# nianticlabs/map-free-reloc

Hardware: AMD Instinct MI355X
Metric: image-pairs/sec @ 540x720 (SuperPoint+SuperGlue + PnP w/ depth) (higher is better)
Workload: dtype f32 in / f32 accumulate; matrix products of the 3x3 convolutions, attention, the transformer's linear layers and SuperPoint's 1x1 descriptor head on the f16 matrix cores with every fp32 operand carried as TWO f16 terms (xh = rne_f16(x), xl = rne_f16((x - xh) 2^11); weights pre-scaled per output feat

## Files before the change

include/mfr_hip.h:

```cpp
#ifndef MFR_HIP_H
#define MFR_HIP_H
#include <stddef.h>
#include <stdint.h>

#ifdef __cplusplus
extern "C" {
#endif

#define MFR_ABI_VERSION 6

#define MFR_K_F32 0
#define MFR_K_F64 1

#define MFR_E_ARG      (-1)
#define MFR_E_LAUNCH   (-2)
#define MFR_E_WORKSPACE (-3)

#define MFR_ST_OK          0
#define MFR_ST_TOO_FEW     1
#define MFR_ST_BAD_DEPTH   2
#define MFR_ST_NO_MODEL    3
#define MFR_ST_DEGENERATE  4

int mfr_abi_version(void);

int mfr_f16x2_guard_bind(int *device_flag);
#define MFR_ST_RANGE 7
const char *mfr_target_arch(void);

int mfr_test_f64_ops(const double *a, const double *b, const double *c, int n, double *out3, void *stream);
int mfr_test_sample(uint64_t seed, const int64_t *pair_ids, int B, int iters, int n, int k, int32_t *out, void *stream);

size_t mfr_pnp_workspace_bytes(int B, int maxN, int max_iters);
int mfr_pnp_solve_batch(const float *pts0, const float *pts1, const int32_t *n_corr, int B, int maxN,
                        const float *depth0, int H, int W,
                        const void *K0, const void *K1, int k_dtype,
                        int max_iters, double reproj_thr, double confidence,
                        uint64_t seed, const int64_t *pair_ids,
                        void *workspace, size_t workspace_bytes,
                        double *R, double *t, int32_t *n_inliers, int32_t *status, uint8_t *inlier_mask,
                        void *stream);

int mfr_depth_min(const float *depth, int B, int H, int W, float *partial_min , void *stream);
int mfr_pnp_lift(const float *pts0, const float *pts1, const int32_t *n_corr, int B, int maxN,
                 const float *depth0, const float *partial_min, int H, int W, const void *K0, int k_dtype,
                 double *xyz, double *obs, int32_t *src_idx, int32_t *n_valid, void *stream);
int mfr_pnp_ransac(const double *xyz, const double *obs, const int32_t *n_valid, int B, int maxN,
                   const void *K1, int k_dtype, int max_iters, double reproj_thr, double confidence,
                   uint64_t seed, const int64_t *pair_ids,
                   int32_t *counts , int32_t *inl_idx ,
                   double *R, double *t, int32_t *n_inliers, int32_t *status,
                   uint8_t *mask_valid ,
                   int32_t *best_iter , int32_t *iters_run ,
                   void *stream);

size_t mfr_rig_pnp_workspace_bytes(int B, int T, int maxN, int max_iters);
int mfr_rig_pnp_ransac(const double *xyz, const double *obs, const int32_t *n_valid, int B, int T, int maxN,
                       const void *K1, int k_dtype, const double *rig, int max_iters, double reproj_thr, double confidence,
                       uint64_t seed, const int64_t *pair_ids,
                       int32_t *counts , int32_t *inl_idx ,
                       double *R, double *t, int32_t *n_inliers, int32_t *status,
                       uint8_t *mask_valid ,
                       int32_t *best_iter , int32_t *iters_run ,
                       void *stream);
int mfr_rig_pnp_solve_batch(const float *pts0, const float *pts1, const int32_t *n_corr, int B, int T, int maxN,
                            const float *depth0, int H, int W,
                            const void *K0, const void *K1, int k_dtype, const double *rig,
                            int max_iters, double reproj_thr, double confidence,
                            uint64_t seed, const int64_t *pair_ids,
                            void *workspace, size_t workspace_bytes,
                            double *R, double *t, int32_t *n_inliers, int32_t *status, uint8_t *inlier_mask ,
                            void *stream);

size_t mfr_scale_workspace_bytes(int B, int maxN);
int mfr_scale_from_depth_batch(const float *pts0, const float *pts1, const uint8_t *emat_mask,
                               const int32_t *n_corr, int B, int maxN,
                               const float *depth0, const float *depth1, int H, int W,
                               const void *K0, const void *K1, int k_dtype,
                               const double *R, const double *t,
                               const int32_t *in_status ,
                               double scale_thr,
                               void *workspace, size_t workspace_bytes,
                               double *t_metric, double *best_scale, int32_t *n_inliers, int32_t *status,
                               void *stream);

#define MFR_AP_OK            0
#define MFR_AP_APPROXIMATED  1
#define MFR_AP_NO_PAIRS      2
#define MFR_AP_TOO_MANY      3
#define MFR_AP_BAD_OFFSETS   4
#define MFR_AP_ITER_CAP      16
#define MFR_AP_MAX_PAIRS     64
#define MFR_AP_MAX_LO_ITERS  62
#define MFR_AP_WEISZFELD_CAP 256
size_t mfr_abs_pose_workspace_bytes(int P);
int mfr_abs_pose_fuse(const double *train_q, const double *train_c, const double *pred_R, const double *pred_t, int P,
                      const int32_t *offsets, int Q, int mode, double thr_deg, double thr_mult, int lo_iters, uint64_t seed,
                      void *workspace, size_t workspace_bytes,
                      double *abs_q, double *abs_c, int32_t *inlier_mask, int32_t *status, void *stream);
int mfr_test_abs_pose_subset(uint64_t seed, const uint64_t *base, int n, int calls, int iters, int nsub, uint64_t *out, void *stream);

#define MFR_EMAT_SCORE_MAGSAC 0
#define MFR_EMAT_SCORE_COUNT  1
#define MFR_MAGSAC_LUT_M 2048
int mfr_magsac_lut(double *lut_host , int M);
size_t mfr_emat_workspace_bytes(int B, int maxN, int max_iters);
int mfr_emat_solve_batch(const float *pts0, const float *pts1, const int32_t *n_corr, int B, int maxN,
                         const void *K0, const void *K1, int k_dtype, double pix_thr, double confidence, int max_iters,
                         uint64_t seed, const int64_t *pair_ids, int score_method, const double *magsac_lut, int lut_m,
                         double max_thr_ratio, void *workspace, size_t workspace_bytes,
                         double *R, double *t, int32_t *n_inliers, int32_t *status, uint8_t *inlier_mask,
                         int32_t *best_iter, int32_t *iters_run, int32_t *counts_out, double *losses_out, int32_t *lo_runs,
                         void *stream);

size_t mfr_procrustes_workspace_bytes(int B, int maxN, int max_iters);
int mfr_procrustes_solve_batch(const float *pts0, const float *pts1, const int32_t *n_corr, int B, int maxN,
                               const float *depth0, const float *depth1, int H, int W, const void *K0, const void *K1, int k_dtype,
                               double max_corr_dist, double confidence, int max_iters, uint64_t seed, const int64_t *pair_ids,
                               void *workspace, size_t workspace_bytes, double *R, double *t, int32_t *n_inliers,
                               int32_t *status, int32_t *best_iter, int32_t *iters_run, int32_t *counts_out, void *stream);

int mfr_sp_scoremap(const float *logits, int B, int Hc, int Wc, float *scores, void *stream);
int mfr_sp_nms_candidates(const float *scores, int B, int H, int W, int nms_radius, float threshold, int border,
                          float *nms_out, uint64_t *cand, int cand_cap, int32_t *cand_count, void *stream);
int mfr_sp_nms_candidates_variant(const float *scores, int B, int H, int W, int nms_radius, float threshold, int border,
                                  float *nms_out, uint64_t *cand, int cand_cap, int32_t *cand_count, int variant, void *stream);
int mfr_sp_nms_stream_geometry(int *useful_cols, int *segment_rows);
int mfr_sp_select_topk(const uint64_t *cand, int cand_cap, const int32_t *cand_count, int B, int W, int K,
                       float *kpts, float *kscores, int32_t *n_kpts, void *stream);
int mfr_sp_sample_descriptors(const float *dense_nhwc, int B, int Hc, int Wc, const float *kpts,
                              const int32_t *n_kpts, int K, float *desc, void *stream);
int mfr_sp_sample_descriptors_ld(const float *dense_nhwc, int B, int Hc, int Wc, const float *kpts,
                                 const int32_t *n_kpts, int K, float *desc, int ldd, void *stream);

size_t mfr_gemm_f16x2_pack_bytes(int N, int K);
int mfr_gemm_f16x2_pack(const float *w, int N, int K, void *packed, void *stream);
int mfr_gemm_f16x2(const float *x, int ldx, const void *packed_w, const float *bias, float *y, int ldy, int M, int N, int K, int flags, void *stream);
int mfr_gemm_f16x2_pack_batched(const float *w, int ldw, int nbatch, long long w_batch_stride, int N, int K, float out_mul, void *packed, void *stream);
int mfr_gemm_f16x2_batched(const float *x, int ldx, long long x_batch_stride, const void *packed_w, const float *bias, float *y, int ldy, long long y_batch_stride,
                           int nbatch, int M, int N, int K, int flags, void *stream);
int mfr_conv_igemm_k(int Cin, int KH, int KW);
int mfr_conv_igemm_f16x2(const float *x, const void *packed_w, const float *bias, float *y, int B, int Cin, int H, int W, int Cout, int KH, int KW,
                         int stride, int pad, int relu, void *stream);
int mfr_conv_igemm_f16x2_pad(const float *x, const void *packed_w, const float *bias, float *y, int B, int Cin, int H, int W, int Cout, int KH, int KW,
                             int stride, int pad_lo, int pad_hi, int relu, void *stream);
int mfr_conv_igemm_f16x2_upadd(const float *x, const void *packed_w, const float *bias, const float *lo, int Hl, int Wl, float *y, int B, int Cin, int H, int W,
                               int Cout, int KH, int KW, int stride, int pad, void *stream);
int mfr_gemm_f16x2_ln(const float *x, int ldx, const void *packed_w, const float *bias, const float *gamma, const float *beta, float eps, float *y, int ldy,
                      int M, int N, int K, int accumulate, void *stream);
int mfr_gemm_bf16x3_ln(const float *x, int ldx, const void *packed_w, const float *bias, const float *gamma, const float *beta, float eps, float *y, int ldy,
                       int M, int N, int K, int accumulate, void *stream);
int mfr_gemm_f16x2_windows(const float *feat, int Bimg, int Hf, int Wf, int C, const int32_t *img_ids, const int32_t *cell_ids, int nwin, int wc, int stride, int win,
                           const float *zero_row, const void *packed_w, const float *bias, const float *window_bias, float *y, int ldy, int N, void *stream);
int mfr_gemm_bf16x3_windows(const float *feat, int Bimg, int Hf, int Wf, int C, const int32_t *img_ids, const int32_t *cell_ids, int nwin, int wc, int stride, int win,
                            const float *zero_row, const void *packed_w, const float *bias, const float *window_bias, float *y, int ldy, int N, void *stream);
int mfr_mlp_ln_f16x2(const float *x, int ldx, int K1, const void *packed_w1, const float *b1, const void *packed_w2, const float *b2, const float *gamma, const float *beta,
                     float eps, float *y, int ldy, int M, int accumulate, void *stream);
int mfr_mlp_ln_bf16x3(const float *x, int ldx, int K1, const void *packed_w1, const float *b1, const void *packed_w2, const float *b2, const float *gamma, const float *beta,
                      float eps, float *y, int ldy, int M, int accumulate, void *stream);
size_t mfr_gemm_bf16x3_pack_bytes(int N, int K);
int mfr_gemm_bf16x3_pack(const float *w, int N, int K, void *packed, void *stream);
int mfr_gemm_bf16x3(const float *x, int ldx, const void *packed_w, const float *bias, float *y, int ldy, int M, int N, int K, int flags, void *stream);
int mfr_sg_attention(const float *q, const float *k, const float *v, int ld, int B2, int N, int heads,
                     const int32_t *n_tok, int cross, float *out, int ldo, void *stream);
int mfr_sg_attention_variant(const float *q, const float *k, const float *v, int ld, int B2, int N, int heads,
                             const int32_t *n_tok, int cross, float *out, int ldo, int variant, void *stream);
size_t mfr_sg_match_workspace_bytes(int B, int ldS);
int mfr_sg_sinkhorn_match(const float *S, int B, int ldS, const int32_t *n0, const int32_t *n1,
                          float bin_score, int iters, float match_thr,
                          const float *kpts0, const float *kpts1, int K,
                          void *workspace, size_t workspace_bytes,
                          int32_t *matches0, float *mscores0, float *pts0, float *pts1, int maxN, int32_t *n_corr,
                          void *stream);
int mfr_sg_sinkhorn_match_variant(const float *S, int B, int ldS, const int32_t *n0, const int32_t *n1,
                                  float bin_score, int iters, float match_thr,
                                  const float *kpts0, const float *kpts1, int K,
                                  void *workspace, size_t workspace_bytes,
                                  int32_t *matches0, float *mscores0, float *pts0, float *pts1, int maxN, int32_t *n_corr,
                                  int variant, void *stream);
int mfr_sg_sinkhorn_match_strided(const float *S, int B, int ldS, const int32_t *n0, const int32_t *n1, long long n_stride,
                                  float bin_score, int iters, float match_thr,
                                  const float *kpts0, const float *kpts1, int K, long long kpts_stride,
                                  void *workspace, size_t workspace_bytes,
                                  int32_t *matches0, float *mscores0, float *pts0, float *pts1, int maxN, int32_t *n_corr,
                                  int variant, void *stream);
int mfr_sg_kenc_in(const float *kpts, const float *scores, const float *w, const float *bias, long long rows, int H, int W, float *out, void *stream);

int mfr_gemm_f16x2_ln_gelu(const float *x, int ldx, const void *packed_w, const float *bias, const float *gamma, const float *beta, float eps, float *y, int ldy,
                           int M, int N, int K, void *stream);
int mfr_gemm_bf16x3_ln_gelu(const float *x, int ldx, const void *packed_w, const float *bias, const float *gamma, const float *beta, float eps, float *y, int ldy,
                            int M, int N, int K, void *stream);
int mfr_lg_rotary_table(const float *kpts_norm, const float *wr, int M, float *cs, void *stream);
int mfr_lg_rotary_apply(float *q, float *k, int ld, int M, const float *cs, void *stream);
int mfr_lg_ln_gelu(float *x, int ld, int M, const float *gamma, const float *beta, float eps, void *stream);
size_t mfr_lg_assign_workspace_bytes(int B, int N0, int N1);
int mfr_lg_assign(const float *S, int B, int N0, int N1, int ldS, const float *z0, const float *z1, const int32_t *n0, const int32_t *n1,
                  float threshold, const float *kpts0, const float *kpts1, int K, void *workspace, size_t workspace_bytes,
                  int32_t *matches0, int32_t *matches1, float *mscores0, float *mscores1, float *pts0, float *pts1, int maxN, int32_t *n_corr,
                  void *stream);

size_t mfr_loftr_linear_attention_workspace_bytes(int B, int L, int heads);
int mfr_loftr_linear_attention(const float *q, int ldq, const float *k, const float *v, int ld, int B, int L, int heads,
                               void *workspace, size_t workspace_bytes, float *out, int ldo, void *stream);
int mfr_loftr_fine_attention(const float *q, int ldq, const float *k, const float *v, int ld, int Bw, int L, int D, int heads,
                             float *out, int ldo, void *stream);
size_t mfr_loftr_coarse_match_workspace_bytes(int B, int L0, int L1);
int mfr_loftr_coarse_match(const float *S, int B, int h0, int w0, int h1, int w1, float temperature, float thr, int border,
                           void *workspace, size_t workspace_bytes, int32_t *i_ids, int32_t *j_ids, float *mconf,
                           int32_t *n_match, void *stream);
int mfr_loftr_coarse_match_variant(const float *S, int B, int h0, int w0, int h1, int w1, float temperature, float thr, int border,
                                   void *workspace, size_t workspace_bytes, int32_t *i_ids, int32_t *j_ids, float *mconf,
                                   int32_t *n_match, int variant, void *stream);
size_t mfr_loftr_ot_match_workspace_bytes(int B, int L0, int L1);
int mfr_loftr_ot_match(const float *S, int B, int h0, int w0, int h1, int w1, float bin_score, int iters, float thr, int border,
                       void *workspace, size_t workspace_bytes, int32_t *i_ids, int32_t *j_ids, float *mconf, int32_t *n_match,
                       float *u_out, float *v_out, int variant, void *stream);
int mfr_loftr_gather_windows(const float *feat, int Bimg, int Hf, int Wf, int C, const int32_t *img_ids,
                             const int32_t *cell_ids, int M, int wc, int stride, int win, float *out, void *stream);
int mfr_loftr_fine_match(const float *g0, const float *g1, int ld, int C, int M, int W, float out_scale, const int32_t *lin_idx,
                         const float *k1, float *pts1, float *expec, void *stream);

int mfr_conv3x3_c1_relu(const float *x, const float *w, const float *bias, int B, int H, int W, int out_channels,
                        float *y, void *stream);
int mfr_bias_relu_nchw(float *x, const float *bias, int B, int C, int HW, void *stream);
int mfr_conv1x1_nchw(const float *x, const float *w, const float *bias, int B, int Cin, int Cout, int HW, float *y, void *stream);
int mfr_nchw_to_rows(const float *x, const float *add, int B, int C, int HW, int deinterleave, float *out, long long out_img_stride, int ldo, void *stream);
int mfr_nchw_to_rows_gather(const float *x, const float *add, int n_src, int C, int HW, const int32_t *idx, int n_out, float *out, long long out_img_stride,
                            int ldo, void *stream);
int mfr_bias_pool2_relu_nchw(const float *x, const float *bias, int B, int C, int H, int W, float *y, void *stream);

size_t mfr_procrustes_icp_workspace_bytes(int B, int H, int W);
int mfr_procrustes_icp_refine(const float *depth0, const float *depth1, int B, int H, int W, const void *K0, const void *K1, int k_dtype,
                              double max_corr_dist, double rel_fitness, double rel_rmse, int max_iter, const int32_t *status,
                              void *workspace, size_t workspace_bytes, double *R, double *t, int32_t *n_inliers, double *fitness,
                              double *rmse, int32_t *iters, void *stream);

int mfr_layernorm(const float *x, int ldx, const float *gamma, const float *beta, const float *residual, int ldr, long long rows, int C,
                  float eps, float *out, int ldo, void *stream);
int mfr_upsample2x_add(const float *lo, float *y, int planes, int H, int W, void *stream);
int mfr_upsample_bilinear(const void *in, void *out, int planes, int H, int W, int Ho, int Wo, int dtype, void *stream);
int mfr_conv_gemm_bf16(const void *A, long long sA, const long long *segA, const void *B, long long sB, const long long *segB,
                       int Lk, int nkc_total, int nkc_z, const float *bias, void *C, long long ldc, int out_dtype,
                       int M, int N, int nz, const long long *zA, const long long *zB, const long long *zC, const int *zk, void *stream);
int mfr_conv_pack_nhwc_halo(const void *x, int x_dtype, int B, int C, int H, int W, int Wp, void *out, int guard_rows, void *stream);
int mfr_conv_pack_cm_halo(const void *x, int x_dtype, long long BC, int H, int W, int Wq, long long L, int ncopies, int first_shift, long long slack,
                          void *out, void *stream);
int mfr_conv_unpack_nchw(const void *haloed, int B, int N, int H, int W, int Wp, void *y, void *stream);

int mfr_kabsch_fwd(const float *H, int B, float *R, void *stream);
int mfr_kabsch_bwd(const float *H, const float *gR, int B, float *gH, void *stream);

int mfr_rootsift(const float *desc, int n_rows, float *out, float *norm2, void *stream);
int mfr_desc_ratio_match(const float *des0, const float *des1, const float *norm0, const float *norm1,
                         const float *kp0, const float *kp1, int B, int N0, int N1,
                         const int32_t *n0, const int32_t *n1, double ratio,
                         int32_t *nn_idx, float *nn_d2, float *pts0, float *pts1, int maxN, int32_t *n_corr,
                         void *stream);

#define MFR_SIFT_ST_CAND_OVERFLOW 1
#define MFR_SIFT_ST_KPT_OVERFLOW  2
#define MFR_SIFT_ST_OUT_OVERFLOW  4
size_t mfr_sift_workspace_bytes(int B, int H, int W, int cand_cap);
long long mfr_sift_level_offset(int B, int H, int W, int octave, int level, int *Ho_host, int *Wo_host);
int mfr_sift_blur_taps(int level, float *taps_host, int *radius_host);
int mfr_sift_detect(const uint8_t *gray, int B, int H, int W, int nfeatures, int Nmax, int cand_cap, void *workspace,
                    size_t workspace_bytes, float *kpts, float *desc, float *size, float *angle, float *response,
                    int32_t *octave, int32_t *n, int32_t *status, void *stream);

size_t mfr_jpeg_workspace_bytes(int n, int H, int W, long long max_record_bytes, int subseq_bits);
int mfr_jpeg_decode(const void *headers, const uint8_t *records, const long long *offsets, int n, int H, int W,
                    long long max_record_bytes, float *gray, uint8_t *rgb, int32_t *status, int32_t *rounds, void *workspace,
                    size_t workspace_bytes, int subseq_bits, void *stream);

size_t mfr_png_depth_workspace_bytes(int n, int H, int W);
int mfr_png_depth_decode(const void *headers, const uint8_t *records, const long long *offsets, int n, int H, int W,
                         long long max_record_bytes, void *scratch, size_t scratch_bytes, float *out, int32_t *status, void *stream);

int mfr_resize_gray_bilinear(const uint8_t *rgb, int n, int H, int W, const int32_t *status,
                             const int32_t *y0, const int32_t *y1, const float *fy,
                             const int32_t *x0, const int32_t *x1, const float *fx,
                             int h, int w, float *out, void *stream);

size_t mfr_wino_f16x2_filter_bytes(int Cin, int Cout);
int mfr_wino_f16x2_filter_transform(const float *w, int Cin, int Cout, void *upk, void *stream);
int mfr_conv3x3_wino_f16x2(const float *x, const void *upk, const float *bias, const float *residual, int B, int Cin, int Cout,
                           int H, int W, int act, int pool, float *y, void *stream);
size_t mfr_conv3x3_direct_f16x2_filter_bytes(int Cin, int Cout);
int mfr_conv3x3_direct_f16x2_filter_pack(const float *w, int Cin, int Cout, void *packed, void *stream);
int mfr_conv3x3_direct_f16x2(const float *x, const void *packed, const float *bias, const float *residual, int B, int Cin, int Cout,
                             int H, int W, int act, int pool, float *y, void *stream);
int mfr_conv3x3_direct_f16x2_rows(const float *x, const void *packed, const float *bias, int B, int Cin, int Cout, int H, int W, int act, float *yrows, int ldy, void *stream);
int mfr_conv3x3_direct_f16x2_tiled(const float *x, const void *packed, const float *bias, const float *residual, int B, int Cin, int Cout, int H, int W,
                                   int act, int pool, float *y, int ldrows, int tile_mode, int pitch, void *stream);
int mfr_conv3x3s2_direct_f16x2(const float *x, const void *packed, const float *bias, int B, int Cin, int Cout, int H, int W, int act, float *y, void *stream);
int mfr_sp_conv1ab_f16x2(const float *gray, const float *w1a, const float *b1a, const void *upk1b, const float *bias1b, int B, int H, int W, float *y, void *stream);
size_t mfr_wino_bf16x3_filter_bytes(int Cin, int Cout);
int mfr_wino_bf16x3_filter_transform(const float *w, int Cin, int Cout, void *upk, void *stream);
int mfr_conv3x3_wino_bf16x3(const float *x, const void *upk, const float *bias, const float *residual, int B, int Cin, int Cout,
                            int H, int W, int act, int pool, float *y, void *stream);
size_t mfr_wino_filter_bytes(int Cin, int Cout);
int mfr_wino_filter_transform(const float *w, int Cin, int Cout, float *upk, void *stream);
int mfr_conv3x3_wino(const float *x, const float *upk, const float *bias, const float *residual, int B, int Cin, int Cout,
                     int H, int W, int act, int pool, float *y, void *stream);
int mfr_conv3x3_wino_variant(const float *x, const float *upk, const float *bias, const float *residual, int B, int Cin, int Cout,
                             int H, int W, int act, int pool, int variant, float *y, void *stream);

int mfr_corr_warp_fwd(const float *q, const float *k, const float *v, const float *grid, int B, int Dq, int N,
                      float *warped, float *pos, float *max_score, float *row_max, float *row_sum, void *stream);
int mfr_corr_warp_bwd(const float *q, const float *k, const float *v, const float *grid, int B, int Dq, int N,
                      const float *d_warped, const float *d_pos, const float *d_max, const float *delta,
                      const float *row_max, const float *row_sum, float *dq, float *dk, float *dv, void *stream);

int mfr_dpt_prep(const void *img, int dtype, int B, int H, int W, float *out, int Hn, int Wn, void *stream);
int mfr_dpt_groupnorm(const float *x, const float *gamma, const float *beta, const float *residual, int B, int C, int HW, int G, float eps, int relu,
                      float *y, void *stream);
int mfr_dpt_maxpool3s2(const float *x, int planes, int H, int W, int pad_top, int pad_bottom, int pad_left, int pad_right, float *y, void *stream);
int mfr_dpt_layernorm(const float *x, int ldx, const float *gamma, const float *beta, const float *residual, int ldr, long long rows, int C, float eps,
                      float *out, int ldo, void *stream);
int mfr_dpt_bias_gelu(float *x, int ld, long long rows, int N, const float *bias, void *stream);
int mfr_dpt_add_relu(const float *a, const float *b, long long n, float *sum, float *relu_out, void *stream);
int mfr_dpt_tokens(const float *x, const float *cls, const float *pos, int B, int C, int HW, float *out, int ldo, void *stream);
int mfr_dpt_tokens_inverse(const float *rows, int ld, long long img_stride, int skip, const float *bias_img, int gelu, int B, int C, int HW, float *out,
                           void *stream);
int mfr_dpt_shuffle(const float *g, int ld, const float *bias, int B, int C, int H, int W, int s, float *out, void *stream);
int mfr_dpt_head_tail(const float *f, const float *w, float bias, int B, int C, int Hh, int Wh, int invert, float scale, float shift, int Ho, int Wo,
                      float *metres, uint16_t *mm, void *stream);
int mfr_dpt_prep_rows(const uint8_t *img, int N, const int *rows, int m, int H, int W, float *out, int Hn, int Wn, int *status, void *stream);
int mfr_dpt_head_tail_rows(const float *f, const float *w, float bias, int B, int C, int Hh, int Wh, int invert, float scale, float shift, int Ho, int Wo,
                           const int *src, const int *dst, int d, float *metres, uint16_t *mm, int D, int quantize, int *status, void *stream);

int mfr_eloftr_stem_s2(const float *x, const float *w, const float *bias, int B, int H, int W, int out_channels, float *y, void *stream);
int mfr_eloftr_aggregate(const float *x, int ldx, long long img_stride, int nimg, int hc, int wc, const float *wq, const float *gamma, const float *beta, float eps,
                         float *q_out, float *kv_out, void *stream);
int mfr_eloftr_rotary(float *q, float *k, int ld, const float *cos_sin, long long rows, int La, void *stream);
int mfr_eloftr_attention(const float *q, int ldq, const float *k, const float *v, int ldkv, int nb, int Lq, int Lk, int heads, float *out, int ldo, void *stream);
int mfr_eloftr_upsample4_rows(const float *msg, int ldm, int nimg, int ha, int wa, float *dst, int ldx, long long img_stride, void *stream);
int mfr_eloftr_upsample2x(const float *in, const float *add, float *out, int planes, int H, int W, void *stream);
int mfr_eloftr_leaky_relu(float *x, int ld, long long rows, int N, float slope, void *stream);
int mfr_eloftr_rows_to_nchw(const float *x, int ldx, long long img_stride, int nimg, int C, int HW, float scale, float *out, void *stream);
int mfr_eloftr_gather_windows(const float *feat_half, int nimg, int Hh, int Wh, int C, const int32_t *img_ids, const int32_t *cell_ids, long long ld_cells,
                              const int32_t *n, int B, int maxN, int wc, int cell_px, int win, int pad, float *out, void *stream);
int mfr_eloftr_fine_match(const float *win0, const float *win1, const int32_t *cell_i, const int32_t *cell_j, long long ld_cells, const int32_t *n, int B, int maxN,
                          int wc, int cell_px, float *pts0, float *pts1, int32_t *stage1_arg, void *stream);
int mfr_eloftr_compact(const float *pts0, const float *pts1, const float *conf, long long ld_conf, const int32_t *n, int B, int maxN, int W, int H, float *out0,
                       float *out1, float *out_conf, int32_t *n_out, void *stream);

int mfr_da_patch_rows(const void *img, int dtype, int B, int H, int W, int gh, int gw, float mean0, float mean1, float mean2, float std0, float std1, float std2,
                      float *rows, int ldk, void *stream);
int mfr_da_patch_rows_tab(const uint8_t *img, int N, const int *tab, int m, int H, int W, int gh, int gw, float mean0, float mean1, float mean2, float std0,
                          float std1, float std2, float *rows, int ldk, int *status, void *stream);
int mfr_da_tokens(const float *x, int ldx, const float *cls, const float *pos, int B, int C, int HW, float *out, int ldo, void *stream);
int mfr_da_head_tail(const float *f, const float *w, float bias, int B, int C, int Hh, int Wh, int metric, float max_depth, int Ho, int Wo, float *metres,
                     uint16_t *mm, void *stream);
int mfr_da_head_tail_rows(const float *f, const float *w, float bias, int B, int C, int Hh, int Wh, int metric, float max_depth, int Ho, int Wo, const int *src,
                          const int *dst, int d, float *metres, uint16_t *mm, int D, int quantize, int *status, void *stream);

#ifdef __cplusplus
}
#endif
#endif
```

map-free-reloc_amd/csrc/gemm_split.hip:

```cpp
#include <hip/hip_runtime.h>
#include <stdint.h>

#include "../../include/mfr_hip.h"
#include "wave_dev.h"
#include "split_f16.h"
#include "guard.h"

using namespace mfr;

typedef short bf16x8 __attribute__((ext_vector_type(8)));
typedef float f32x16 __attribute__((ext_vector_type(16)));

#define GB_BM 128
#define GB_BN 128
#define GB_BK 32
#define GB_KG_STRIDE 129
#define GB_TERM_UNITS (4 * GB_KG_STRIDE)
#define GB_WT(F16) ((F16) ? 2 : 3)
#define GB_W_TILE_UNITS(F16) (GB_WT(F16) * 512)

union GbFrag { bf16x8 v; unsigned u[4]; uint4 q; };

typedef _Float16 gb_h8 __attribute__((ext_vector_type(8)));
__device__ __forceinline__ uint4 gb_wq(const uint4 &wh)
{
    const gb_h8 h = __builtin_bit_cast(gb_h8, wh);
    const gb_h8 q = h * (_Float16)(1.0f / SF_LOW_SCALE);
    return __builtin_bit_cast(uint4, q);
}

template <bool F16>
__device__ __forceinline__ void gb_xsplit_store(uint4 *lds, const float4 &p, const float4 &q, int dst)
{
    if (F16) {
        unsigned h[4], l[4];
        sf_split2(p.x, p.y, SF_LOW_SCALE, h[0], l[0]); sf_split2(p.z, p.w, SF_LOW_SCALE, h[1], l[1]);
        sf_split2(q.x, q.y, SF_LOW_SCALE, h[2], l[2]); sf_split2(q.z, q.w, SF_LOW_SCALE, h[3], l[3]);
        lds[0 * GB_TERM_UNITS + dst] = make_uint4(h[0], h[1], h[2], h[3]);
        lds[1 * GB_TERM_UNITS + dst] = make_uint4(l[0], l[1], l[2], l[3]);
    } else {
        const float x[8] = { p.x, p.y, p.z, p.w, q.x, q.y, q.z, q.w };
        unsigned h[8], m[8], l[8];
#pragma unroll
        for (int e = 0; e < 8; ++e) bf_split3(x[e], h[e], m[e], l[e]);
        lds[0 * GB_TERM_UNITS + dst] = make_uint4(bf_pack_hi16(h[0], h[1]), bf_pack_hi16(h[2], h[3]), bf_pack_hi16(h[4], h[5]), bf_pack_hi16(h[6], h[7]));
        lds[1 * GB_TERM_UNITS + dst] = make_uint4(bf_pack_hi16(m[0], m[1]), bf_pack_hi16(m[2], m[3]), bf_pack_hi16(m[4], m[5]), bf_pack_hi16(m[6], m[7]));
        lds[2 * GB_TERM_UNITS + dst] = make_uint4(bf_pack_hi16(l[0], l[1]), bf_pack_hi16(l[2], l[3]), bf_pack_hi16(l[4], l[5]), bf_pack_hi16(l[6], l[7]));
    }
}

#define GB_MFMA_BF(a, b, c) __builtin_amdgcn_mfma_f32_32x32x16_bf16((a), (b), (c), 0, 0, 0)
template <bool F16, bool SWAP>
__device__ __forceinline__ void gb_products(f32x16 (&acc)[2][2], const GbFrag (&a)[2][3], const GbFrag (&b)[2][3])
{
#define GB_P4(ta, tb) do { \
        _Pragma("unroll") for (int i = 0; i < 2; ++i) \
            _Pragma("unroll") for (int j = 0; j < 2; ++j) { \
                const GbFrag &p = SWAP ? b[i][tb] : a[i][ta], &q = SWAP ? a[j][ta] : b[j][tb]; \
                if (F16) acc[i][j] = SF_MFMA(p.q, q.q, acc[i][j]); else acc[i][j] = GB_MFMA_BF(p.v, q.v, acc[i][j]); } } while (0)
    if (F16) { GB_P4(1, 2); GB_P4(0, 1); GB_P4(0, 0); }
    else     { GB_P4(1, 1); GB_P4(0, 2); GB_P4(2, 0); GB_P4(0, 1); GB_P4(1, 0); GB_P4(0, 0); }
#undef GB_P4
}
#define GB_XT(F16) ((F16) ? 2 : 3)

#define GB_ACC_ROW(i, r) (32 * (i) + ((r) & 3) + 8 * ((r) >> 2))
#define GB_TILE_ROW(base, i, r) ((base) + 32 * (i) + ((r) & 3) + 8 * ((r) >> 2) + 4 * (lane >> 5))
#define GB_FRAG_ROW(w, kg_stride) ((lane >> 5) * (kg_stride) + 64 * (w) + (lane & 31))
#define GB_XSTAGE() \
    int xdst[2], xr[2], xk[2]; \
    _Pragma("unroll") for (int i = 0; i < 2; ++i) { \
        const int u = tid + 256 * i; \
        xr[i] = u >> 2; xk[i] = 8 * (u & 3); \
        xdst[i] = (u & 3) * GB_KG_STRIDE + xr[i]; \
    }
#define GB_XSRC(mb, i) (X + (size_t)min((mb) * GB_BM + xr[i], M - 1) * ldx + xk[i])
__device__ __forceinline__ int gb_wdst(int tid, int i, int xt)
{
    const int u = tid + 256 * i, term = u / 512, kg = (u % 512) / 128, f = u % 128;
    return (xt + term) * GB_TERM_UNITS + kg * GB_KG_STRIDE + f;
}
#define GB_WIDX_REG ((XT + t) * GB_TERM_UNITS + 2 * ks * GB_KG_STRIDE + brow + 32 * i)
#define GB_MMA_KSTEP(acc, SWAP, WIDX) do { \
        _Pragma("unroll") for (int ks = 0; ks < 2; ++ks) { \
            GbFrag a[2][3], b[2][3]; \
            _Pragma("unroll") for (int i = 0; i < 2; ++i) { \
                _Pragma("unroll") for (int t = 0; t < XT; ++t) a[i][t].q = lds[t * GB_TERM_UNITS + 2 * ks * GB_KG_STRIDE + arow + 32 * i]; \
                _Pragma("unroll") for (int t = 0; t < WT; ++t) b[i][t].q = lds[WIDX]; \
                if (F16) b[i][2].q = gb_wq(b[i][0].q); } \
            gb_products<F16, SWAP>(acc, a, b); } } while (0)
#define GB_ZERO(acc) do { \
        _Pragma("unroll") for (int i = 0; i < 2; ++i) \
            _Pragma("unroll") for (int jj = 0; jj < 2; ++jj) \
                _Pragma("unroll") for (int r = 0; r < 16; ++r) acc[i][jj][r] = 0.f; } while (0)
#define GB_GUARD_ROWS(acc, chk) do { \
        _Pragma("unroll") for (int i = 0; i < 2; ++i) \
            _Pragma("unroll") for (int r = 0; r < 16; ++r) MFR_GUARD_ACC(chk, acc[i][0][r]); \
        mfr_guard_commit(guard, chk); } while (0)
#define GB_BATCH_OFFSETS() do { const size_t bz_ = blockIdx.y; X += bz_ * (size_t)xs; Wp += bz_ * (size_t)ws; Y += bz_ * (size_t)ys; if (F16) oscale += bz_ * (size_t)ws * 4; } while (0)

__global__ void __launch_bounds__(64) gb_scale_kernel(const float *__restrict__ w, int N, int K, int npad, float *__restrict__ oscale, float out_mul,
                                                      int ldw, long long w_stride, long long p_stride_f)
{
    w += (size_t)blockIdx.y * (size_t)w_stride; oscale += (size_t)blockIdx.y * (size_t)p_stride_f;
    const int n = blockIdx.x, lane = threadIdx.x;
    float mx = 0.f;
    if (n < N)
        for (int k = lane; k < K; k += 64) mx = fmaxf(mx, fabsf(w[(size_t)n * ldw + k]));
    mx = wave_max(mx);
    if (lane == 0 && n < npad) oscale[n] = out_mul / sf_feature_scale(mx);
}
template <bool F16>
__global__ void __launch_bounds__(256) gb_pack_kernel(const float *__restrict__ w, int N, int K, long long total, const float *__restrict__ oscale, uint4 *__restrict__ out,
                                                      float out_mul, int ldw, long long w_stride, long long p_stride_u)
{
    w += (size_t)blockIdx.y * (size_t)w_stride; out += (size_t)blockIdx.y * (size_t)p_stride_u;
    if (F16) oscale += (size_t)blockIdx.y * (size_t)p_stride_u * 4;
    const long long t = (long long)blockIdx.x * 256 + threadIdx.x;
    if (t >= total) return;
    const int u = (int)(t % GB_W_TILE_UNITS(F16));
    const long long tile = t / GB_W_TILE_UNITS(F16);
    const int nkb = K / GB_BK;
    const int kb = (int)(tile % nkb), nb = (int)(tile / nkb);
    const int term = u / 512, kg = (u % 512) / 128, f = u % 128;
    const int n = nb * GB_BN + f, k0 = kb * GB_BK + 8 * kg;
    unsigned word[8];
    const float s = F16 ? out_mul / oscale[n] : 1.0f;
#pragma unroll
    for (int e = 0; e < 8; ++e) {
        const float x = (n < N) ? w[(size_t)n * ldw + k0 + e] : 0.f;
        if (F16) {
            unsigned short wh, wl, wq;
            sf_split_w(x * s, wh, wl, wq);
            (void)wq;
            word[e] = (unsigned)(term == 0 ? wh : wl) << 16;
        } else {
            unsigned h, m, l;
            bf_split3(x, h, m, l);
            word[e] = term == 0 ? h : term == 1 ? m : l;
        }
    }
    out[t] = make_uint4(bf_pack_hi16(word[0], word[1]), bf_pack_hi16(word[2], word[3]), bf_pack_hi16(word[4], word[5]), bf_pack_hi16(word[6], word[7]));
}

template <int FLAGS, bool F16>
__global__ void __launch_bounds__(256, 2) gemm_split_kernel(const float *__restrict__ X, int ldx, const uint4 *__restrict__ Wp, const float *__restrict__ oscale,
                                                            const float *__restrict__ bias, float *__restrict__ Y, int ldy, int M, int N, int K, int nnb,
                                                            long long xs, long long ws, long long ys, int *guard)
{
    GB_BATCH_OFFSETS();
    constexpr int XT = GB_XT(F16);
    constexpr int WT = GB_WT(F16);
    __shared__ uint4 lds[(XT + WT) * GB_TERM_UNITS];
    const int tid = threadIdx.x, lane = tid & 63, wid = tid >> 6;
    const int wm = wid >> 1, wn = wid & 1;
    const int nb = blockIdx.x % nnb, mb = blockIdx.x / nnb;
    const int m0 = mb * GB_BM;
    const int nkb = K / GB_BK;

    const float *xrow[2];
    int xdst[2];
#pragma unroll
    for (int i = 0; i < 2; ++i) {
        const int u = tid + 256 * i, row = u >> 2, kg = u & 3;
        const int m = min(m0 + row, M - 1);
        xrow[i] = X + (size_t)m * ldx + 8 * kg;
        xdst[i] = kg * GB_KG_STRIDE + row;
    }
    int wdst[2 * WT];
#pragma unroll
    for (int i = 0; i < 2 * WT; ++i) wdst[i] = gb_wdst(tid, i, XT);
    const uint4 *wtile = Wp + (size_t)nb * nkb * GB_W_TILE_UNITS(F16) + tid;

    float4 xa0, xa1, xb0, xb1;
    uint4 w0, w1, w2, w3, w4, w5;
#define GB_GLOAD(kb) do { \
        xa0 = *(const float4 *)(xrow[0] + (kb) * GB_BK); xa1 = *(const float4 *)(xrow[0] + (kb) * GB_BK + 4); \
        xb0 = *(const float4 *)(xrow[1] + (kb) * GB_BK); xb1 = *(const float4 *)(xrow[1] + (kb) * GB_BK + 4); \
        const uint4 *wt_ = wtile + (size_t)(kb) * GB_W_TILE_UNITS(F16); \
        w0 = wt_[0]; w1 = wt_[256]; w2 = wt_[512]; w3 = wt_[768]; if (WT == 3) { w4 = wt_[1024]; w5 = wt_[1280]; } } while (0)

    f32x16 acc[2][2];
    GB_ZERO(acc);
    const int arow = GB_FRAG_ROW(wm, GB_KG_STRIDE);
    const int brow = GB_FRAG_ROW(wn, GB_KG_STRIDE);

    GB_GLOAD(0);
    for (int kb = 0; kb < nkb; ++kb) {
        __syncthreads();
        gb_xsplit_store<F16>(lds, xa0, xa1, xdst[0]); gb_xsplit_store<F16>(lds, xb0, xb1, xdst[1]);
        lds[wdst[0]] = w0; lds[wdst[1]] = w1; lds[wdst[2]] = w2; lds[wdst[3]] = w3;
        if (WT == 3) { lds[wdst[2 * WT - 2]] = w4; lds[wdst[2 * WT - 1]] = w5; }
        __syncthreads();
        { const int kn = min(kb + 1, nkb - 1); GB_GLOAD(kn); }
        __builtin_amdgcn_sched_barrier(0);
        GB_MMA_KSTEP(acc, false, GB_WIDX_REG);
    }
#undef GB_GLOAD

    if (F16 && guard) { float chk = 0.f; GB_GUARD_ROWS(acc, chk); }
#pragma unroll
    for (int j = 0; j < 2; ++j) {
        const int n = nb * GB_BN + 64 * wn + 32 * j + (lane & 31);
        if (n >= N) continue;
        const float bv = bias ? bias[n] : 0.f;
        const float os = F16 ? oscale[n] : 1.0f;
#pragma unroll
        for (int i = 0; i < 2; ++i) {
#pragma unroll
            for (int r = 0; r < 16; ++r) {
                const int m = GB_TILE_ROW(m0 + 64 * wm, i, r);
                if (m >= M) continue;
                float *yp = Y + (size_t)m * ldy + n;
                float v = F16 ? __builtin_fmaf(acc[i][j][r], os, bv) : acc[i][j][r] + bv;
                if (FLAGS & 1) v = fmaxf(v, 0.f);
                if (FLAGS & 2) v += *yp;
                *yp = v;
            }
        }
    }
}

#define GB_TILE(j, mb_, nb_) const int nb_ = (j) % nnb, mb_ = ((j) / nnb) * 8 + xcd
#define GB_WALK() \
    const int xcd = blockIdx.x & 7, slot = blockIdx.x >> 3, per_xcd = gridDim.x >> 3; \
    const int items = ((nmb + 7) >> 3) * nnb; \
    int j = slot; \
    if (j >= items) return; \
    { GB_TILE(j, mb, nb); (void)nb; if (mb >= nmb) return; }
#define GB_WALK_NEXT() \
    auto next_item = [&](int jj) { int jn = jj + per_xcd; if (jn < items) { GB_TILE(jn, mbn, nbn); (void)nbn; if (mbn >= nmb) jn = items; } return jn < items ? jn : jj; }
#define GB_YTILE(nb) \
    const __amdgpu_buffer_rsrc_t ry = __builtin_amdgcn_make_buffer_rsrc((void *)(Y + (size_t)m0 * ldy), 0, (int)((unsigned)min(GB_BM, M - m0) * rowb), MFR_RSRC_FLAGS); \
    const int n0 = (nb) * GB_BN + 64 * wn + (lane & 31); \
    const unsigned yoff = (unsigned)(64 * wm + 4 * (lane >> 5)) * rowb + 4u * (unsigned)n0
#define GB_SOFF(i, r) ((unsigned)GB_ACC_ROW(i, r) * rowb)
#define GB_PREFETCH_Y() do { \
        _Pragma("unroll") for (int jj = 0; jj < 2; ++jj) \
            _Pragma("unroll") for (int i = 0; i < 2; ++i) \
                _Pragma("unroll") for (int r = 0; r < 16; ++r) \
                    ov[i][jj][r] = __builtin_amdgcn_raw_buffer_load_b32(ry, yoff + 128u * jj, GB_SOFF(i, r), 0); } while (0)
#define GB_COLS() \
    const __amdgpu_buffer_rsrc_t rbias = __builtin_amdgcn_make_buffer_rsrc((void *)bias, 0, bias ? N * 4 : 0, MFR_RSRC_FLAGS); \
    const __amdgpu_buffer_rsrc_t rscale = __builtin_amdgcn_make_buffer_rsrc((void *)oscale, 0, F16 ? nnb * GB_BN * 4 : 0, MFR_RSRC_FLAGS)
#define GB_COLS_LOAD() \
    const float bv0 = __builtin_bit_cast(float, __builtin_amdgcn_raw_buffer_load_b32(rbias, 4u * (unsigned)n0, 0, 0)); \
    const float bv1 = __builtin_bit_cast(float, __builtin_amdgcn_raw_buffer_load_b32(rbias, 4u * (unsigned)n0 + 128u, 0, 0)); \
    const float os0 = __builtin_bit_cast(float, __builtin_amdgcn_raw_buffer_load_b32(rscale, 4u * (unsigned)n0, 0, 0)); \
    const float os1 = __builtin_bit_cast(float, __builtin_amdgcn_raw_buffer_load_b32(rscale, 4u * (unsigned)n0 + 128u, 0, 0))
__device__ __forceinline__ void gb_xload(const float *&lx0, const float *&lx1, float4 &p0, float4 &p1, float4 &q0, float4 &q1)
{
    p0 = *(const float4 *)lx0; p1 = *(const float4 *)(lx0 + 4); q0 = *(const float4 *)lx1; q1 = *(const float4 *)(lx1 + 4);
    lx0 += GB_BK; lx1 += GB_BK;
}
#define GB_NO_ROW_BIAS(v, i, jj, r) (void)0
#define GB_STORE_PLAIN(acc, ROW_BIAS) do { \
        _Pragma("unroll") for (int jj = 0; jj < 2; ++jj) { \
            if (n0 + 32 * jj >= N) continue; \
            const float bv = jj ? bv1 : bv0, os = jj ? os1 : os0; \
            _Pragma("unroll") for (int i = 0; i < 2; ++i) \
                _Pragma("unroll") for (int r = 0; r < 16; ++r) { \
                    float v = F16 ? __builtin_fmaf(acc[i][jj][r], os, bv) : acc[i][jj][r] + bv; \
                    if (FLAGS & 1) v = fmaxf(v, 0.f); \
                    if (FLAGS & 2) v += __builtin_bit_cast(float, ov[i][jj][r]); \
                    ROW_BIAS(v, i, jj, r); \
                    __builtin_amdgcn_raw_buffer_store_b32(__builtin_bit_cast(unsigned, v), ry, yoff + 128u * jj, GB_SOFF(i, r), 0); \
                } } } while (0)
#define GB_LN_ROW_SUMS(at) do { \
        _Pragma("unroll") for (int m = 1; m <= 16; m <<= 1) \
            _Pragma("unroll") for (int i = 0; i < 2; ++i) \
                _Pragma("unroll") for (int r = 0; r < 16; ++r) part[i][r] += __shfl_xor(part[i][r], m, 64); \
        if ((lane & 31) == 0) { \
            _Pragma("unroll") for (int i = 0; i < 2; ++i) \
                _Pragma("unroll") for (int r = 0; r < 16; ++r) lnx[(at) + wn * 128 + GB_TILE_ROW(64 * wm, i, r)] = part[i][r]; \
        } \
        __syncthreads(); } while (0)
#define GB_STORE_LAYERNORM(acc, ACCUMULATE, B0, B1, S0, S1) do { \
        float part[2][16]; \
        _Pragma("unroll") for (int i = 0; i < 2; ++i) \
            _Pragma("unroll") for (int r = 0; r < 16; ++r) { \
                acc[i][0][r] = F16 ? __builtin_fmaf(acc[i][0][r], S0, B0) : acc[i][0][r] + B0; \
                acc[i][1][r] = F16 ? __builtin_fmaf(acc[i][1][r], S1, B1) : acc[i][1][r] + B1; \
                part[i][r] = acc[i][0][r] + acc[i][1][r]; \
            } \
        GB_LN_ROW_SUMS(0); \
        _Pragma("unroll") for (int i = 0; i < 2; ++i) \
            _Pragma("unroll") for (int r = 0; r < 16; ++r) { \
                const float mean = (lnx[GB_TILE_ROW(64 * wm, i, r)] + lnx[128 + GB_TILE_ROW(64 * wm, i, r)]) * (1.0f / 128.0f); \
                acc[i][0][r] -= mean; acc[i][1][r] -= mean; \
                part[i][r] = acc[i][0][r] * acc[i][0][r] + acc[i][1][r] * acc[i][1][r]; \
            } \
        GB_LN_ROW_SUMS(256); \
        _Pragma("unroll") for (int i = 0; i < 2; ++i) \
            _Pragma("unroll") for (int r = 0; r < 16; ++r) { \
                const float rstd = rsqrtf((lnx[256 + GB_TILE_ROW(64 * wm, i, r)] + lnx[384 + GB_TILE_ROW(64 * wm, i, r)]) * (1.0f / 128.0f) + ln_eps); \
                float y0 = acc[i][0][r] * rstd * g0 + be0, y1 = acc[i][1][r] * rstd * g1 + be1; \
                if (ACCUMULATE) { y0 = __builtin_bit_cast(float, ov[i][0][r]) + y0; y1 = __builtin_bit_cast(float, ov[i][1][r]) + y1; } \
                __builtin_amdgcn_raw_buffer_store_b32(__builtin_bit_cast(unsigned, y0), ry, yoff, GB_SOFF(i, r), 0); \
                __builtin_amdgcn_raw_buffer_store_b32(__builtin_bit_cast(unsigned, y1), ry, yoff + 128u, GB_SOFF(i, r), 0); \
            } } while (0)

template <int FLAGS, bool F16>
__global__ void __launch_bounds__(256, 2) gemm_split_pk_kernel(const float *__restrict__ X, int ldx, const uint4 *__restrict__ Wp, const float *__restrict__ oscale,
                                                               const float *__restrict__ bias, float *__restrict__ Y, int ldy, int M, int N, int K, int nnb, int nmb,
                                                               long long xs, long long ws, long long ys, int *guard)
{
    GB_BATCH_OFFSETS();
    constexpr int XT = GB_XT(F16);
    constexpr int WT = GB_WT(F16);
    __shared__ uint4 lds[(XT + WT) * GB_TERM_UNITS];
    const int tid = threadIdx.x, lane = tid & 63, wid = tid >> 6;
    const int wm = wid >> 1, wn = wid & 1;
    const int nkb = K / GB_BK;
    GB_WALK();

    GB_XSTAGE();
    int wdst[2 * WT];
#pragma unroll
    for (int i = 0; i < 2 * WT; ++i) wdst[i] = gb_wdst(tid, i, XT);
    const int arow = GB_FRAG_ROW(wm, GB_KG_STRIDE);
    const int brow = GB_FRAG_ROW(wn, GB_KG_STRIDE);
    const unsigned rowb = (unsigned)ldy * 4u;
    GB_COLS();

    const float *lx0, *lx1;
    const uint4 *lw;
    int lk, lj = j;
    auto load_tile_start = [&](int jj) {
        GB_TILE(jj, mb, nb);
        lx0 = GB_XSRC(mb, 0);
        lx1 = GB_XSRC(mb, 1);
        lw = Wp + (size_t)nb * nkb * GB_W_TILE_UNITS(F16) + tid;
        lk = 0;
    };
    float4 xa0, xa1, xb0, xb1;
    uint4 w0, w1, w2, w3, w4, w5;
#define GB_PLOAD() do { \
        xa0 = *(const float4 *)lx0; xa1 = *(const float4 *)(lx0 + 4); xb0 = *(const float4 *)lx1; xb1 = *(const float4 *)(lx1 + 4); \
        w0 = lw[0]; w1 = lw[256]; w2 = lw[512]; w3 = lw[768]; if (WT == 3) { w4 = lw[1024]; w5 = lw[1280]; } \
        lx0 += GB_BK; lx1 += GB_BK; lw += GB_W_TILE_UNITS(F16); \
        if (++lk == nkb) { int jn = lj + per_xcd; if (jn < items) { GB_TILE(jn, mbn_, nbn_); (void)nbn_; if (mbn_ >= nmb) jn = items; } \
                           if (jn < items) lj = jn; load_tile_start(lj); } } while (0)

    f32x16 acc[2][2];
    unsigned ov[2][2][16];

    load_tile_start(j);
    GB_PLOAD();
    for (;;) {
        GB_TILE(j, mb, nb);
        const int m0 = mb * GB_BM;
        GB_YTILE(nb);
        GB_COLS_LOAD();
        GB_ZERO(acc);
#define GB_PSTEP(LAST) do { \
            __syncthreads(); \
            gb_xsplit_store<F16>(lds, xa0, xa1, xdst[0]); gb_xsplit_store<F16>(lds, xb0, xb1, xdst[1]); \
            lds[wdst[0]] = w0; lds[wdst[1]] = w1; lds[wdst[2]] = w2; lds[wdst[3]] = w3; \
            if (WT == 3) { lds[wdst[2 * WT - 2]] = w4; lds[wdst[2 * WT - 1]] = w5; } \
            __syncthreads(); \
            GB_PLOAD(); \
            if ((LAST) && (FLAGS & 2)) GB_PREFETCH_Y(); \
            __builtin_amdgcn_sched_barrier(0); \
            GB_MMA_KSTEP(acc, false, GB_WIDX_REG); } while (0)
        for (int kb = 0; kb < nkb - 1; ++kb) GB_PSTEP(false);
        GB_PSTEP(true);

        if (F16 && guard) { float chk = 0.f; GB_GUARD_ROWS(acc, chk); }
        GB_STORE_PLAIN(acc, GB_NO_ROW_BIAS);
        int jn = j + per_xcd;
        if (jn >= items) break;
        { GB_TILE(jn, mbn, nbn); (void)nbn; if (mbn >= nmb) break; }
        j = jn;
    }
#undef GB_PSTEP
#undef GB_PLOAD
}

#define GD_WSTAGE(F16) GB_W_TILE_UNITS(F16)
#define GD_VMCNT(n) __builtin_amdgcn_s_waitcnt(0x0F70 | ((n) & 15) | (((n) >> 4) << 14))
#ifdef GD_PROF
__device__ unsigned long long gd_prof[4][64];
#define GD_STAMP(k) do { if (blockIdx.x == (gridDim.x / 2 | 3u) && lane == 0 && pstep < 12) { __builtin_amdgcn_sched_barrier(0); gd_prof[wid][5 * pstep + (k)] = __builtin_amdgcn_s_memtime(); __builtin_amdgcn_sched_barrier(0); } } while (0)
#else
#define GD_STAMP(k) do { } while (0)
#endif
typedef unsigned gd_u32x4 __attribute__((ext_vector_type(4)));
#define GD_WDESC(wdesc, Wp, wp_bytes) \
    gd_u32x4 wdesc; \
    wdesc.x = __builtin_amdgcn_readfirstlane((unsigned)(unsigned long long)Wp); \
    wdesc.y = __builtin_amdgcn_readfirstlane((unsigned)((unsigned long long)Wp >> 32) & 0xffffu); \
    wdesc.z = wp_bytes; \
    wdesc.w = MFR_RSRC_FLAGS
#define GD_WDMA_LANE() \
    const unsigned lds0 = (unsigned)(unsigned long long)(__attribute__((address_space(3))) uint4 *)lds; \
    const unsigned lane16 = 16u * (unsigned)lane
#define GD_WDMA_LOAD(wdesc) asm volatile("s_mov_b32 m0, %0\n\ts_nop 0\n\tbuffer_load_dwordx4 %1, %2, %3 offen lds" :: "s"(m0v), "v"(lane16), "s"(wdesc), "s"(so) : "memory")
#define GD_WDMA_ISSUE(img, stage, LOAD) do { \
        _Pragma("unroll") for (int q = 0; q < 2 * WT; ++q) { \
            const unsigned so = __builtin_amdgcn_readfirstlane(img + (unsigned)(64 * (wid + 4 * q)) * 16u); \
            const unsigned m0v = __builtin_amdgcn_readfirstlane(lds0 + 16u * (unsigned)(XT * GB_TERM_UNITS + stage * WSTAGE + 64 * (wid + 4 * q))); \
            LOAD; \
        } } while (0)
#define GD_WIDX(P) ((P) * WSTAGE + t * 512 + 2 * ks * 128 + brow + 32 * i)
struct GdWindows {
    const int *img_ids, *cell_ids;
    const float *zero;
    const float *rgb;
    int wc, stride, Hf, Wf, win;
};

template <int FLAGS, bool F16>
__global__ void __launch_bounds__(256, 2) gemm_split_d_kernel(const float *__restrict__ X, int ldx, const uint4 *__restrict__ Wp, unsigned wp_bytes, const float *__restrict__ oscale,
                                                              const float *__restrict__ bias, float *__restrict__ Y, int ldy, int M, int N, int K, int nnb, int nmb,
                                                              long long xs, long long ws, long long ys, int *guard,
                                                              const float *__restrict__ ln_gamma, const float *__restrict__ ln_beta, float ln_eps, GdWindows wnd)
{
    GB_BATCH_OFFSETS();
    constexpr int XT = GB_XT(F16);
    constexpr int WT = GB_WT(F16), WSTAGE = GD_WSTAGE(F16);
    __shared__ uint4 lds[XT * GB_TERM_UNITS + 2 * WSTAGE];
    __shared__ float lnx[(FLAGS & 4) ? 512 : 1];
    const int tid = threadIdx.x, lane = tid & 63, wid = __builtin_amdgcn_readfirstlane(tid >> 6);
    const int wm = wid >> 1, wn = wid & 1;
    const int nkb = K / GB_BK;
    GB_WALK();
    GB_WALK_NEXT();

    GB_XSTAGE();
    const int arow = GB_FRAG_ROW(wm, GB_KG_STRIDE);
    const int brow = XT * GB_TERM_UNITS + GB_FRAG_ROW(wn, 128);
    const unsigned rowb = (unsigned)ldy * 4u;
    GB_COLS();

    GD_WDESC(wdesc, Wp, wp_bytes);
    GD_WDMA_LANE();
    int wj = j, wk = 0;
    auto wdma = [&](int stage) {
        GB_TILE(wj, mbw, nbw); (void)mbw;
        const unsigned img = (unsigned)(nbw * nkb + wk) * (unsigned)(WSTAGE * 16);
        GD_WDMA_ISSUE(img, stage, GD_WDMA_LOAD(wdesc));
        if (++wk == nkb) { wk = 0; wj = next_item(wj); }
    };
    const float *lx0, *lx1;
    int lk = 0, lj = j;
    auto window_row = [&](int g) -> const float * {
        const int ww = wnd.win * wnd.win, m = g / ww, t = g - m * ww, ky = t / wnd.win;
        const int img = wnd.img_ids[m], cell = wnd.cell_ids[m];
        const int y = (cell / wnd.wc) * wnd.stride - wnd.win / 2 + ky, x = (cell % wnd.wc) * wnd.stride - wnd.win / 2 + (t - ky * wnd.win);
        return (y >= 0 && y < wnd.Hf && x >= 0 && x < wnd.Wf) ? X + (((size_t)img * wnd.Hf + y) * wnd.Wf + x) * (size_t)ldx : wnd.zero;
    };
    auto x_tile_start = [&](int jj) {
        GB_TILE(jj, mb, nb); (void)nb;
        if constexpr ((FLAGS & 8) != 0) {
            lx0 = window_row(min(mb * GB_BM + xr[0], M - 1)) + xk[0];
            lx1 = window_row(min(mb * GB_BM + xr[1], M - 1)) + xk[1];
        } else {
            lx0 = GB_XSRC(mb, 0);
            lx1 = GB_XSRC(mb, 1);
        }
    };
    float4 xa0, xa1, xb0, xb1, xc0, xc1, xd0, xd1;
#define GD_XLOAD(p0, p1, q0, q1) do { \
        gb_xload(lx0, lx1, p0, p1, q0, q1); \
        if (++lk == nkb) { lk = 0; lj = next_item(lj); x_tile_start(lj); } } while (0)

    f32x16 acc[2][2];
    unsigned ov[2][2][16];
#ifdef GD_PROF
    int pstep = 0;
#define GD_PSTEP_INC ++pstep
#else
#define GD_PSTEP_INC (void)0
#endif
#define GD_STEP(P, p0, p1, q0, q1, LAST) do { \
        GD_STAMP(0); \
        __syncthreads(); \
        GD_STAMP(1); \
        gb_xsplit_store<F16>(lds, p0, p1, xdst[0]); gb_xsplit_store<F16>(lds, q0, q1, xdst[1]); \
        wdma((P) ^ 1); GD_XLOAD(p0, p1, q0, q1); \
        GD_STAMP(2); \
        if ((LAST) && (FLAGS & 2)) { GB_PREFETCH_Y(); GD_VMCNT(63); } \
        else GD_VMCNT(8 + 2 * WT); \
        GD_STAMP(3); \
        __syncthreads(); \
        GD_STAMP(4); \
        __builtin_amdgcn_sched_barrier(0); \
        GB_MMA_KSTEP(acc, false, GD_WIDX(P)); \
        GD_PSTEP_INC; } while (0)

    x_tile_start(j);
    wdma(0);
    GD_XLOAD(xa0, xa1, xb0, xb1);
    GD_XLOAD(xc0, xc1, xd0, xd1);
    for (;;) {
        GB_TILE(j, mb, nb);
        const int m0 = mb * GB_BM;
        GB_YTILE(nb);
        GB_COLS_LOAD();
        GB_ZERO(acc);
        for (int kb = 0; kb < nkb - 2; kb += 2) { GD_STEP(0, xa0, xa1, xb0, xb1, false); GD_STEP(1, xc0, xc1, xd0, xd1, false); }
        GD_STEP(0, xa0, xa1, xb0, xb1, false);
        GD_STEP(1, xc0, xc1, xd0, xd1, true);
        if (F16 && guard) { float chk = 0.f; GB_GUARD_ROWS(acc, chk); }
        if constexpr ((FLAGS & 4) != 0) {
            const float g0 = ln_gamma[n0], g1 = ln_gamma[n0 + 32], be0 = ln_beta[n0], be1 = ln_beta[n0 + 32];
            GB_STORE_LAYERNORM(acc, FLAGS & 2, bv0, bv1, os0, os1);
        } else {
#define GD_WINDOW_BIAS(v, i, jj, r) \
            if constexpr ((FLAGS & 8) != 0) { \
                if (wnd.rgb) { \
                    const int g = min(GB_TILE_ROW(m0 + 64 * wm, i, r), M - 1); \
                    v += wnd.rgb[(size_t)(g / (wnd.win * wnd.win)) * N + n0 + 32 * jj]; \
                } \
            }
            GB_STORE_PLAIN(acc, GD_WINDOW_BIAS);
#undef GD_WINDOW_BIAS
        }
        const int jn = next_item(j);
        if (jn == j) break;
        j = jn;
    }
    GD_VMCNT(0);
#undef GD_STEP
#undef GD_XLOAD
}

static __device__ __forceinline__ void gb_swap32(float &a, float &b) { asm("s_nop 1\n\tv_permlane32_swap_b32 %0, %1" : "+v"(a), "+v"(b)); }

template <bool F16, bool ACC>
__global__ void __launch_bounds__(256, 2) mlp_ln_kernel(const float *__restrict__ X, int ldx, int K1,
                                                        const uint4 *__restrict__ W1p, unsigned w1_bytes, const float *__restrict__ os1, const float *__restrict__ b1,
                                                        const uint4 *__restrict__ W2p, unsigned w2_bytes, const float *__restrict__ os2, const float *__restrict__ b2,
                                                        const float *__restrict__ ln_gamma, const float *__restrict__ ln_beta, float ln_eps,
                                                        float *__restrict__ Y, int ldy, int M, int nmb, int *guard)
{
    constexpr int XT = GB_XT(F16);
    constexpr int WT = GB_WT(F16), WSTAGE = GD_WSTAGE(F16);
    __shared__ uint4 lds[XT * GB_TERM_UNITS + 2 * WSTAGE];
    __shared__ float lnx[512];
    const int tid = threadIdx.x, lane = tid & 63, wid = __builtin_amdgcn_readfirstlane(tid >> 6);
    const int wm = wid >> 1, wn = wid & 1;
    const int nkb1 = K1 / GB_BK;
    const int half_steps = nkb1 + 4, steps = 2 * half_steps;
    constexpr int nnb = 1;
    GB_WALK();
    GB_WALK_NEXT();

    GB_XSTAGE();
    const int arow = GB_FRAG_ROW(wm, GB_KG_STRIDE);
    const int brow = XT * GB_TERM_UNITS + GB_FRAG_ROW(wn, 128);
    const unsigned rowb = (unsigned)ldy * 4u;

    GD_WDESC(wdesc1, W1p, w1_bytes);
    GD_WDESC(wdesc2, W2p, w2_bytes);
    GD_WDMA_LANE();
    int wstep = 0;
    auto wdma = [&](int stage) {
        const int half = wstep >= half_steps ? 1 : 0, r = wstep - half * half_steps;
        const bool first = r < nkb1;
        const unsigned img = (unsigned)(first ? half * nkb1 + r : 4 * half + (r - nkb1)) * (unsigned)(WSTAGE * 16);
        GD_WDMA_ISSUE(img, stage, if (first) GD_WDMA_LOAD(wdesc1); else GD_WDMA_LOAD(wdesc2));
        if (++wstep == steps) wstep = 0;
    };
    const float *lx0, *lx1;
    int xstep = 0, lj = j;
    auto x_tile_start = [&](int jj) {
        GB_TILE(jj, mb, nb); (void)nb;
        lx0 = GB_XSRC(mb, 0);
        lx1 = GB_XSRC(mb, 1);
    };
    float4 xa0, xa1, xb0, xb1, xc0, xc1, xd0, xd1;
#define ML_XLOAD(p0, p1, q0, q1) do { \
        gb_xload(lx0, lx1, p0, p1, q0, q1); ++xstep; \
        if (xstep == nkb1) { lx0 -= K1; lx1 -= K1; } \
        else if (xstep == 2 * nkb1) { xstep = 0; lj = next_item(lj); x_tile_start(lj); } } while (0)

    f32x16 acc1[2][2], acc2[2][2];
#define ML_STEP1(P, p0, p1, q0, q1, FIRST) do { \
        __syncthreads(); \
        gb_xsplit_store<F16>(lds, p0, p1, xdst[0]); gb_xsplit_store<F16>(lds, q0, q1, xdst[1]); \
        wdma((P) ^ 1); ML_XLOAD(p0, p1, q0, q1); \
        if (FIRST) GD_VMCNT(4 + 2 * WT); else GD_VMCNT(8 + 2 * WT); \
        __syncthreads(); \
        __builtin_amdgcn_sched_barrier(0); \
        GB_MMA_KSTEP(acc1, true, GD_WIDX(P)); } while (0)

    x_tile_start(j);
    wdma(0);
    ML_XLOAD(xa0, xa1, xb0, xb1);
    ML_XLOAD(xc0, xc1, xd0, xd1);
    const float g0 = ln_gamma[64 * wn + (lane & 31)], g1 = ln_gamma[64 * wn + 32 + (lane & 31)];
    const float be0 = ln_beta[64 * wn + (lane & 31)], be1 = ln_beta[64 * wn + 32 + (lane & 31)];
    for (;;) {
        GB_TILE(j, mb, nb);
        const int m0 = mb * GB_BM;
        GB_YTILE(nb);
        GB_ZERO(acc2);
        float chk = 0.f;
        for (int h = 0; h < 2; ++h) {
            GB_ZERO(acc1);
            ML_STEP1(0, xa0, xa1, xb0, xb1, true);
            ML_STEP1(1, xc0, xc1, xd0, xd1, false);
            for (int kb = 2; kb < nkb1; kb += 2) { ML_STEP1(0, xa0, xa1, xb0, xb1, false); ML_STEP1(1, xc0, xc1, xd0, xd1, false); }
            if (F16 && guard) { MFR_GUARD_ACC(chk, acc1[0][0][0]); MFR_GUARD_ACC(chk, acc1[0][1][0]); }
#pragma unroll
            for (int fi = 0; fi < 2; ++fi)
#pragma unroll
                for (int r = 0; r < 16; ++r) {
                    const int f = GB_TILE_ROW(128 * h + 64 * wn, fi, r);
                    const float bv = b1 ? b1[f] : 0.f;
                    const float os = F16 ? os1[f] : 1.0f;
#pragma unroll
                    for (int rj = 0; rj < 2; ++rj) {
                        const float v = F16 ? __builtin_fmaf(acc1[fi][rj][r], os, bv) : acc1[fi][rj][r] + bv;
                        acc1[fi][rj][r] = fmaxf(v, 0.f);
                    }
                }
#pragma unroll
            for (int fi = 0; fi < 2; ++fi)
#pragma unroll
                for (int rj = 0; rj < 2; ++rj)
#pragma unroll
                    for (int r = 0; r < 8; ++r) {
                        float a_ = acc1[fi][rj][r], b_ = acc1[fi][rj][r + 8];
                        gb_swap32(a_, b_);
                        acc1[fi][rj][r] = a_; acc1[fi][rj][r + 8] = b_;
                    }
#pragma unroll
            for (int c = 0; c < 4; ++c) {
                __syncthreads();
                if (wn == (c >> 1)) {
                    const int fi = c & 1;
#pragma unroll
                    for (int rj = 0; rj < 2; ++rj)
#pragma unroll
                        for (int gq = 0; gq < 2; ++gq) {
                            const float4 p = make_float4(acc1[fi][rj][4 * gq], acc1[fi][rj][4 * gq + 1], acc1[fi][rj][4 * gq + 2], acc1[fi][rj][4 * gq + 3]);
                            const float4 q = make_float4(acc1[fi][rj][8 + 4 * gq], acc1[fi][rj][9 + 4 * gq], acc1[fi][rj][10 + 4 * gq], acc1[fi][rj][11 + 4 * gq]);
                            gb_xsplit_store<F16>(lds, p, q, (gq + 2 * (lane >> 5)) * GB_KG_STRIDE + 64 * wm + 32 * rj + (lane & 31));
                        }
                }
                wdma((c & 1) ^ 1);
                GD_VMCNT(2 * WT);
                __syncthreads();
                __builtin_amdgcn_sched_barrier(0);
                GB_MMA_KSTEP(acc2, false, GD_WIDX(c & 1));
            }
        }
        unsigned ov[2][2][16];
        if (ACC) GB_PREFETCH_Y();
        if (F16 && guard) GB_GUARD_ROWS(acc2, chk);
        {
            const float bv0 = b2 ? b2[n0] : 0.f, bv1 = b2 ? b2[n0 + 32] : 0.f;
            const float os0 = F16 ? os2[n0] : 1.f, os1v = F16 ? os2[n0 + 32] : 1.f;
            GB_STORE_LAYERNORM(acc2, ACC, bv0, bv1, os0, os1v);
        }
        const int jn = next_item(j);
        if (jn == j) break;
        j = jn;
    }
    GD_VMCNT(0);
#undef ML_STEP1
#undef ML_XLOAD
}

template <bool F16>
__global__ void __launch_bounds__(256, 1) gemm_ln512_gelu_kernel(const float *__restrict__ X, int ldx, const uint4 *__restrict__ Wp, const float *__restrict__ oscale,
                                                                 const float *__restrict__ bias, const float *__restrict__ ln_gamma, const float *__restrict__ ln_beta,
                                                                 float ln_eps, float *__restrict__ Y, int ldy, int M, int K, int *guard)
{
    constexpr int XT = GB_XT(F16);
    constexpr int WT = GB_WT(F16);
    __shared__ uint4 lds[(XT + 4 * WT) * GB_TERM_UNITS];
    __shared__ float lnx[512];
    const int tid = threadIdx.x, lane = tid & 63, wid = tid >> 6;
    const int wm = wid >> 1, wn = wid & 1;
    const int m0 = blockIdx.x * GB_BM;
    const int nkb = K / GB_BK;

    const float *xrow[2];
    int xdst[2];
#pragma unroll
    for (int i = 0; i < 2; ++i) {
        const int u = tid + 256 * i, row = u >> 2, kg = u & 3;
        const int m = min(m0 + row, M - 1);
        xrow[i] = X + (size_t)m * ldx + 8 * kg;
        xdst[i] = kg * GB_KG_STRIDE + row;
    }
    int wdst[2 * WT];
#pragma unroll
    for (int i = 0; i < 2 * WT; ++i) wdst[i] = gb_wdst(tid, i, XT);
    const int arow = GB_FRAG_ROW(wm, GB_KG_STRIDE);
    const int brow = GB_FRAG_ROW(wn, GB_KG_STRIDE);

    float4 xa0, xa1, xb0, xb1;
    uint4 w00, w01, w02, w03, w04, w05, w10, w11, w12, w13, w14, w15, w20, w21, w22, w23, w24, w25, w30, w31, w32, w33, w34, w35;
#define GL_WLOAD(q, kb) do { \
        const uint4 *wt_ = Wp + ((size_t)(q) * nkb + (kb)) * GB_W_TILE_UNITS(F16) + tid; \
        w##q##0 = wt_[0]; w##q##1 = wt_[256]; w##q##2 = wt_[512]; w##q##3 = wt_[768]; if (WT == 3) { w##q##4 = wt_[1024]; w##q##5 = wt_[1280]; } } while (0)
#define GL_WSTORE(q) do { \
        uint4 *ld_ = lds + (q) * WT * GB_TERM_UNITS; \
        ld_[wdst[0]] = w##q##0; ld_[wdst[1]] = w##q##1; ld_[wdst[2]] = w##q##2; ld_[wdst[3]] = w##q##3; \
        if (WT == 3) { ld_[wdst[2 * WT - 2]] = w##q##4; ld_[wdst[2 * WT - 1]] = w##q##5; } } while (0)
#define GL_GLOAD(kb) do { \
        xa0 = *(const float4 *)(xrow[0] + (kb) * GB_BK); xa1 = *(const float4 *)(xrow[0] + (kb) * GB_BK + 4); \
        xb0 = *(const float4 *)(xrow[1] + (kb) * GB_BK); xb1 = *(const float4 *)(xrow[1] + (kb) * GB_BK + 4); \
        GL_WLOAD(0, kb); GL_WLOAD(1, kb); GL_WLOAD(2, kb); GL_WLOAD(3, kb); } while (0)
#define GL_WIDX ((XT + WT * q + t) * GB_TERM_UNITS + 2 * ks * GB_KG_STRIDE + brow + 32 * i)

    f32x16 acc[4][2][2];
#pragma unroll
    for (int q = 0; q < 4; ++q) GB_ZERO(acc[q]);
    GL_GLOAD(0);
    for (int kb = 0; kb < nkb; ++kb) {
        __syncthreads();
        gb_xsplit_store<F16>(lds, xa0, xa1, xdst[0]); gb_xsplit_store<F16>(lds, xb0, xb1, xdst[1]);
        GL_WSTORE(0); GL_WSTORE(1); GL_WSTORE(2); GL_WSTORE(3);
        __syncthreads();
        { const int kn = min(kb + 1, nkb - 1); GL_GLOAD(kn); }
        __builtin_amdgcn_sched_barrier(0);
#pragma unroll
        for (int q = 0; q < 4; ++q) GB_MMA_KSTEP(acc[q], false, GL_WIDX);
    }
#undef GL_WIDX
#undef GL_GLOAD
#undef GL_WLOAD
#undef GL_WSTORE

    if (F16 && guard) { float chk = 0.f; GB_GUARD_ROWS(acc[0], chk); }
    const int nl = 64 * wn + (lane & 31);
    float part[2][16];
#pragma unroll
    for (int i = 0; i < 2; ++i)
#pragma unroll
        for (int r = 0; r < 16; ++r) part[i][r] = 0.f;
#pragma unroll
    for (int nb = 0; nb < 4; ++nb)
#pragma unroll
        for (int jj = 0; jj < 2; ++jj) {
            const int n = 128 * nb + nl + 32 * jj;
            const float bv = bias ? bias[n] : 0.f, os = F16 ? oscale[n] : 1.0f;
#pragma unroll
            for (int i = 0; i < 2; ++i)
#pragma unroll
                for (int r = 0; r < 16; ++r) {
                    acc[nb][i][jj][r] = F16 ? __builtin_fmaf(acc[nb][i][jj][r], os, bv) : acc[nb][i][jj][r] + bv;
                    part[i][r] += acc[nb][i][jj][r];
                }
        }
    GB_LN_ROW_SUMS(0);
#pragma unroll
    for (int i = 0; i < 2; ++i)
#pragma unroll
        for (int r = 0; r < 16; ++r) {
            const float mean = (lnx[GB_TILE_ROW(64 * wm, i, r)] + lnx[128 + GB_TILE_ROW(64 * wm, i, r)]) * (1.0f / 512.0f);
            float sq = 0.f;
#pragma unroll
            for (int nb = 0; nb < 4; ++nb)
#pragma unroll
                for (int jj = 0; jj < 2; ++jj) { acc[nb][i][jj][r] -= mean; sq += acc[nb][i][jj][r] * acc[nb][i][jj][r]; }
            part[i][r] = sq;
        }
    GB_LN_ROW_SUMS(256);
    float rstd[2][16];
#pragma unroll
    for (int i = 0; i < 2; ++i)
#pragma unroll
        for (int r = 0; r < 16; ++r)
            rstd[i][r] = rsqrtf((lnx[256 + GB_TILE_ROW(64 * wm, i, r)] + lnx[384 + GB_TILE_ROW(64 * wm, i, r)]) * (1.0f / 512.0f) + ln_eps);
#pragma unroll
    for (int nb = 0; nb < 4; ++nb)
#pragma unroll
        for (int jj = 0; jj < 2; ++jj) {
            const int n = 128 * nb + nl + 32 * jj;
            const float g = ln_gamma[n], be = ln_beta[n];
#pragma unroll
            for (int i = 0; i < 2; ++i)
#pragma unroll
                for (int r = 0; r < 16; ++r) {
                    const int m = GB_TILE_ROW(m0 + 64 * wm, i, r);
                    if (m >= M) continue;
                    const float u = acc[nb][i][jj][r] * rstd[i][r] * g + be;
                    Y[(size_t)m * ldy + n] = 0.5f * u * (1.0f + erff(u * 0.70710678118654752440f));
                }
        }
}

template <int MODE, bool RELU, bool UP>
__global__ void __launch_bounds__(256, 2) conv_igemm_f16x2_kernel(const float *__restrict__ X, const uint4 *__restrict__ Wp, const float *__restrict__ oscale,
                                                                  const float *__restrict__ bias, float *__restrict__ Y, int B, int Cin, int H, int W, int Cout,
                                                                  int Ho, int Wo, int KH, int KW, int stride, int pad, int nkb, int cblocks, int nnb, int npt, int *guard,
                                                                  const float *__restrict__ lo, int Hl, int Wl, float rh, float rw)
{
    constexpr int XT = 2, WT = 2;
    __shared__ uint4 lds[(XT + WT) * GB_TERM_UNITS];
    const int tid = threadIdx.x, lane = tid & 63, wid = __builtin_amdgcn_readfirstlane(tid >> 6);
    const int wm = wid >> 1, wn = wid & 1;
    const int nb = blockIdx.x % nnb;
    const int pt = (blockIdx.x / nnb) % npt, b = blockIdx.x / (nnb * npt);
    const int HW = H * W, HoWo = Ho * Wo;
    const __amdgpu_buffer_rsrc_t rx = __builtin_amdgcn_make_buffer_rsrc((void *)(X + (size_t)b * Cin * HW), 0, Cin * HW * 4, MFR_RSRC_FLAGS);

    int xdst[2], kg[2];
    int iy0[2], ix0[2];
    {
        const int p = pt * 128 + (tid & 127);
        const int oy = p / Wo, ox = p - oy * Wo;
        const bool pv = p < HoWo;
#pragma unroll
        for (int i = 0; i < 2; ++i) {
            kg[i] = __builtin_amdgcn_readfirstlane((tid >> 7) + 2 * i);
            xdst[i] = kg[i] * GB_KG_STRIDE + (tid & 127);
            iy0[i] = pv ? oy * stride - pad : -(1 << 20);
            ix0[i] = ox * stride - pad;
        }
    }
    int wdst[2 * WT];
#pragma unroll
    for (int i = 0; i < 2 * WT; ++i) wdst[i] = gb_wdst(tid, i, XT);
    const uint4 *wtile = Wp + (size_t)nb * nkb * GB_W_TILE_UNITS(true) + tid;

    float xr[2][8];
    uint4 w0, w1, w2, w3;
    auto gload = [&](int kb) {
        if (MODE == 0) {
            const int tap = kb / cblocks, c0 = (kb - tap * cblocks) * 32;
            const int dy = tap / KW, dx = tap - dy * KW;
            const int iy = iy0[0] + dy, ix = ix0[0] + dx;
            const unsigned vo = (iy >= 0 && iy < H && ix >= 0 && ix < W) ? (unsigned)(iy * W + ix) * 4u : 0x80000000u;
#pragma unroll
            for (int i = 0; i < 2; ++i)
#pragma unroll
                for (int e = 0; e < 8; ++e) {
                    const int ch = c0 + 8 * kg[i] + e;
                    xr[i][e] = __builtin_bit_cast(float, __builtin_amdgcn_raw_buffer_load_b32(rx, ch < Cin ? vo : 0x80000000u, (unsigned)min(ch, Cin - 1) * (unsigned)HW * 4u, 0));
                }
        } else {
#pragma unroll
            for (int i = 0; i < 2; ++i)
#pragma unroll
                for (int e = 0; e < 8; ++e) {
                    const int tap = kb * 32 + 8 * kg[i] + e;
                    const int dy = tap / KW, dx = tap - dy * KW;
                    const int iy = iy0[0] + dy, ix = ix0[0] + dx;
                    const unsigned vo = (tap < KH * KW && iy >= 0 && iy < H && ix >= 0 && ix < W) ? (unsigned)(iy * W + ix) * 4u : 0x80000000u;
                    xr[i][e] = __builtin_bit_cast(float, __builtin_amdgcn_raw_buffer_load_b32(rx, vo, 0, 0));
                }
        }
        const uint4 *wt_ = wtile + (size_t)kb * GB_W_TILE_UNITS(true);
        w0 = wt_[0]; w1 = wt_[256]; w2 = wt_[512]; w3 = wt_[768];
    };
    auto lstore = [&]() {
#pragma unroll
        for (int i = 0; i < 2; ++i) {
            unsigned h[4], l[4];
#pragma unroll
            for (int q = 0; q < 4; ++q) sf_split2(xr[i][2 * q], xr[i][2 * q + 1], SF_LOW_SCALE, h[q], l[q]);
            lds[0 * GB_TERM_UNITS + xdst[i]] = make_uint4(h[0], h[1], h[2], h[3]);
            lds[1 * GB_TERM_UNITS + xdst[i]] = make_uint4(l[0], l[1], l[2], l[3]);
        }
        lds[wdst[0]] = w0; lds[wdst[1]] = w1; lds[wdst[2]] = w2; lds[wdst[3]] = w3;
    };

    f32x16 acc[2][2];
    GB_ZERO(acc);
    const int wrow = GB_FRAG_ROW(wm, GB_KG_STRIDE);
    const int prow = GB_FRAG_ROW(wn, GB_KG_STRIDE);

    gload(0);
    for (int kb = 0; kb < nkb; ++kb) {
        __syncthreads();
        lstore();
        __syncthreads();
        gload(min(kb + 1, nkb - 1));
        __builtin_amdgcn_sched_barrier(0);
#pragma unroll
        for (int ks = 0; ks < 2; ++ks) {
            uint4 wh[2], wl[2], xh[2], xl[2];
#pragma unroll
            for (int i = 0; i < 2; ++i) {
                wh[i] = lds[(XT + 0) * GB_TERM_UNITS + 2 * ks * GB_KG_STRIDE + wrow + 32 * i];
                wl[i] = lds[(XT + 1) * GB_TERM_UNITS + 2 * ks * GB_KG_STRIDE + wrow + 32 * i];
                xh[i] = lds[0 * GB_TERM_UNITS + 2 * ks * GB_KG_STRIDE + prow + 32 * i];
                xl[i] = lds[1 * GB_TERM_UNITS + 2 * ks * GB_KG_STRIDE + prow + 32 * i];
            }
#pragma unroll
            for (int i = 0; i < 2; ++i) {
                const uint4 wq = gb_wq(wh[i]);
#pragma unroll
                for (int j = 0; j < 2; ++j) acc[i][j] = SF_MFMA(wq, xl[j], acc[i][j]);
            }
#pragma unroll
            for (int i = 0; i < 2; ++i)
#pragma unroll
                for (int j = 0; j < 2; ++j) acc[i][j] = SF_MFMA(wl[i], xh[j], acc[i][j]);
#pragma unroll
            for (int i = 0; i < 2; ++i)
#pragma unroll
                for (int j = 0; j < 2; ++j) acc[i][j] = SF_MFMA(wh[i], xh[j], acc[i][j]);
        }
    }

    if (guard) {
        float chk = 0.f;
        MFR_GUARD_ACC(chk, acc[0][0][0]); MFR_GUARD_ACC(chk, acc[0][1][0]);
        mfr_guard_commit(guard, chk);
    }
    const __amdgpu_buffer_rsrc_t rsY = __builtin_amdgcn_make_buffer_rsrc((void *)(Y + (size_t)b * Cout * HoWo), 0, Cout * HoWo * 4, MFR_RSRC_FLAGS);
    const __amdgpu_buffer_rsrc_t rsL = __builtin_amdgcn_make_buffer_rsrc((void *)(UP ? lo + (size_t)b * Cout * ((size_t)Hl * Wl) : nullptr), 0, UP ? Cout * Hl * Wl * 4 : 0, MFR_RSRC_FLAGS);
    float osv[2][16], bvv[2][16];
    unsigned cho[2][16];
#pragma unroll
    for (int i = 0; i < 2; ++i)
#pragma unroll
        for (int r = 0; r < 16; ++r) {
            const int co = GB_TILE_ROW(nb * GB_BN + 64 * wm, i, r);
            osv[i][r] = oscale[co];
            bvv[i][r] = bias ? bias[min(co, Cout - 1)] : 0.f;
            cho[i][r] = co < Cout ? (unsigned)co : 0x10000000u;
        }
    unsigned pixoff[2];
    unsigned uo[2], udw[2], udh[2];
    float uh0[2], uh1[2], uw0[2], uw1[2];
#pragma unroll
    for (int j = 0; j < 2; ++j) {
        const int p = pt * 128 + 64 * wn + 32 * j + (lane & 31);
        pixoff[j] = p < HoWo ? (unsigned)p * 4u : 0x80000000u;
        if (UP) {
            const int pc = min(p, HoWo - 1);
            const int oy = pc / Wo, ox = pc - oy * Wo;
            const float h1r = rh * oy, w1r = rw * ox;
            const int h1 = min((int)h1r, Hl - 1), w1 = min((int)w1r, Wl - 1);
            uh1[j] = h1r - h1; uh0[j] = 1.f - uh1[j];
            uw1[j] = w1r - w1; uw0[j] = 1.f - uw1[j];
            uo[j] = (unsigned)(h1 * Wl + w1) * 4u; udw[j] = (w1 < Wl - 1) ? 4u : 0u; udh[j] = (h1 < Hl - 1) ? (unsigned)Wl * 4u : 0u;
        }
    }
    const unsigned HlWl4 = (unsigned)(Hl * Wl) * 4u, HoWo4 = (unsigned)HoWo * 4u;
    constexpr int UD = 2;
    float ut[UP ? 32 : 1][2][4];
    auto uload = [&](int it) {
        if (UP) {
            const int i = it >> 4, r = it & 15;
            const unsigned cb = cho[i][r] < 0x10000000u ? cho[i][r] * HlWl4 : 0x80000000u;
#pragma unroll
            for (int j = 0; j < 2; ++j) {
                ut[it][j][0] = __builtin_bit_cast(float, __builtin_amdgcn_raw_buffer_load_b32(rsL, cb + uo[j], 0, 0));
                ut[it][j][1] = __builtin_bit_cast(float, __builtin_amdgcn_raw_buffer_load_b32(rsL, cb + uo[j] + udw[j], 0, 0));
                ut[it][j][2] = __builtin_bit_cast(float, __builtin_amdgcn_raw_buffer_load_b32(rsL, cb + uo[j] + udh[j], 0, 0));
                ut[it][j][3] = __builtin_bit_cast(float, __builtin_amdgcn_raw_buffer_load_b32(rsL, cb + uo[j] + udh[j] + udw[j], 0, 0));
            }
        }
    };
    if (UP) {
#pragma unroll
        for (int it = 0; it < UD; ++it) uload(it);
    }
#pragma unroll
    for (int it = 0; it < 32; ++it) {
        const int i = it >> 4, r = it & 15;
        if (UP && it + UD < 32) uload(it + UD);
        const unsigned cb = cho[i][r] < 0x10000000u ? cho[i][r] * HoWo4 : 0x40000000u;
#pragma unroll
        for (int j = 0; j < 2; ++j) {
            float v = __builtin_fmaf(acc[i][j][r], osv[i][r], bvv[i][r]);
            if (RELU) v = fmaxf(v, 0.f);
            if (UP) v += uh0[j] * (uw0[j] * ut[it][j][0] + uw1[j] * ut[it][j][1]) + uh1[j] * (uw0[j] * ut[it][j][2] + uw1[j] * ut[it][j][3]);
            __builtin_amdgcn_raw_buffer_store_b32(__builtin_bit_cast(unsigned, v), rsY, cb + pixoff[j], 0, 0);
        }
    }
}

static size_t gb_tile_bytes(int N, int K, bool f16) { return (size_t)((N + GB_BN - 1) / GB_BN) * (K / GB_BK) * GB_W_TILE_UNITS(f16) * 16; }

template <bool F16>
struct GbOperand {
    const uint4 *wp;
    size_t tb;
    const float *oscale;
    GbOperand(const void *packed_w, int N, int K) : wp((const uint4 *)packed_w), tb(gb_tile_bytes(N, K, F16)), oscale(F16 ? (const float *)((const char *)packed_w + tb) : nullptr) {}
    bool dma_ok() const { return tb < 0xffffffffull; }
    static int *guard() { return F16 ? mfr_guard_current() : (int *)nullptr; }
};
static unsigned gb_persistent_grid(int nmb, int nnb, long long cap = 64)
{
    const long long per_xcd = (long long)((nmb + 7) / 8) * nnb;
    return 8u * (unsigned)(per_xcd < cap ? per_xcd : cap);
}
template <int FLAGS, bool F16>
static void gb_launch_d(hipStream_t st, unsigned grid, const float *x, int ldx, const GbOperand<F16> &w, const float *bias, float *y, int ldy, int M, int N, int K,
                        int nbatch = 1, long long xs = 0, long long ws = 0, long long ys = 0, const float *ln_gamma = nullptr, const float *ln_beta = nullptr,
                        float ln_eps = 0.f, const GdWindows &wnd = GdWindows{})
{
    hipLaunchKernelGGL((gemm_split_d_kernel<FLAGS, F16>), dim3(grid, (unsigned)nbatch), dim3(256), 0, st, x, ldx, w.wp, (unsigned)w.tb, w.oscale, bias, y, ldy, M, N, K,
                       (N + GB_BN - 1) / GB_BN, (M + GB_BM - 1) / GB_BM, xs, ws, ys, GbOperand<F16>::guard(), ln_gamma, ln_beta, ln_eps, wnd);
}

template <bool F16>
static int gb_launch(const float *x, int ldx, const void *packed_w, const float *bias, float *y, int ldy, int M, int N, int K, int flags, void *stream,
                     int nbatch = 1, long long xs = 0, long long ws_bytes = 0, long long ys = 0, const float *ln_gamma = nullptr, const float *ln_beta = nullptr,
                     float ln_eps = 0.f)
{
    hipStream_t st = (hipStream_t)stream;
    if (ln_gamma) {
        if (!ln_beta || N != GB_BN || (K % 64) || (flags & ~2) || nbatch != 1 || !x || !packed_w || !y || M <= 0 || (ldx & 3) || ldx < K || ldy < N || ((uintptr_t)x & 15)) return MFR_E_ARG;
        const GbOperand<F16> w(packed_w, N, K);
        if (!w.dma_ok()) return MFR_E_ARG;
        const unsigned grid = gb_persistent_grid((M + GB_BM - 1) / GB_BM, 1);
        if (flags & 2) gb_launch_d<6, F16>(st, grid, x, ldx, w, bias, y, ldy, M, N, K, 1, 0, 0, 0, ln_gamma, ln_beta, ln_eps);
        else           gb_launch_d<4, F16>(st, grid, x, ldx, w, bias, y, ldy, M, N, K, 1, 0, 0, 0, ln_gamma, ln_beta, ln_eps);
        CHECK_LAUNCH();
        return 0;
    }
    if (nbatch <= 0 || nbatch > 65535 || (ws_bytes & 15) || (xs & 3) || xs < 0 || ys < 0) return MFR_E_ARG;
    const long long ws = ws_bytes / 16;
    if (!x || !packed_w || !y || M <= 0 || N <= 0 || K <= 0 || (K % GB_BK) || (ldx & 3) || ldx < K || ldy < N || flags < 0 || (flags & ~15) || (flags & 12) == 12) return MFR_E_ARG;
    if (((uintptr_t)x & 15)) return MFR_E_ARG;
    const int f = flags & 3, one_tile = flags & 4;
    int pk = flags & 8;
    const GbOperand<F16> w(packed_w, N, K);
    if (!one_tile && !pk && ((K % 64) || !w.dma_ok())) pk = 8;
    const int nnb = (N + GB_BN - 1) / GB_BN, nmb = (M + GB_BM - 1) / GB_BM;
    const long long tiles = (long long)nmb * nnb;
    if (tiles > 0x7fffffffll) return MFR_E_ARG;
    const unsigned grid = gb_persistent_grid(nmb, nnb, (F16 && !(f & 2) && !pk) ? 96 : 64);
#define GB_SW(GO) switch (f) { case 0: GO(0); break; case 1: GO(1); break; case 2: GO(2); break; default: GO(3); break; }
    if (one_tile) {
#define GB_GO(F) hipLaunchKernelGGL((gemm_split_kernel<F, F16>), dim3((unsigned)tiles, (unsigned)nbatch), dim3(256), 0, st, x, ldx, w.wp, w.oscale, bias, y, ldy, M, N, K, nnb, xs, ws, ys, w.guard())
        GB_SW(GB_GO)
#undef GB_GO
    } else if (pk) {
#define GB_GO(F) hipLaunchKernelGGL((gemm_split_pk_kernel<F, F16>), dim3(grid, (unsigned)nbatch), dim3(256), 0, st, x, ldx, w.wp, w.oscale, bias, y, ldy, M, N, K, nnb, nmb, xs, ws, ys, w.guard())
        GB_SW(GB_GO)
#undef GB_GO
    } else {
#define GB_GO(F) gb_launch_d<F, F16>(st, grid, x, ldx, w, bias, y, ldy, M, N, K, nbatch, xs, ws, ys)
        GB_SW(GB_GO)
#undef GB_GO
    }
#undef GB_SW
    CHECK_LAUNCH();
    return 0;
}

template <bool F16>
static int gb_mlp_ln(const float *x, int ldx, int K1, const void *packed_w1, const float *b1, const void *packed_w2, const float *b2, const float *gamma, const float *beta,
                     float eps, float *y, int ldy, int M, int accumulate, void *stream)
{
    if (!x || !packed_w1 || !packed_w2 || !gamma || !beta || !y || M <= 0 || K1 <= 0 || (K1 % 64) || (ldx & 3) || ldx < K1 || ldy < GB_BN || ((uintptr_t)x & 15)) return MFR_E_ARG;
    const GbOperand<F16> w1(packed_w1, 2 * GB_BN, K1), w2(packed_w2, GB_BN, 2 * GB_BN);
    if (!w1.dma_ok()) return MFR_E_ARG;
    const int nmb = (M + GB_BM - 1) / GB_BM;
    const unsigned grid = gb_persistent_grid(nmb, 1);
#define GB_GO(A) hipLaunchKernelGGL((mlp_ln_kernel<F16, A>), dim3(grid), dim3(256), 0, (hipStream_t)stream, x, ldx, K1, w1.wp, (unsigned)w1.tb, w1.oscale, b1, \
                                    w2.wp, (unsigned)w2.tb, w2.oscale, b2, gamma, beta, eps, y, ldy, M, nmb, w1.guard())
    if (accumulate) GB_GO(true); else GB_GO(false);
#undef GB_GO
    CHECK_LAUNCH();
    return 0;
}

template <bool F16>
static int gb_ln_gelu(const float *x, int ldx, const void *packed_w, const float *bias, const float *gamma, const float *beta, float eps, float *y, int ldy,
                      int M, int N, int K, void *stream)
{
    if (!x || !packed_w || !gamma || !beta || !y || M <= 0 || N != 4 * GB_BN || K <= 0 || (K % GB_BK) || (ldx & 3) || ldx < K || ldy < N || !(eps >= 0.f) ||
        ((uintptr_t)x & 15)) return MFR_E_ARG;
    const GbOperand<F16> w(packed_w, N, K);
    hipLaunchKernelGGL((gemm_ln512_gelu_kernel<F16>), dim3((unsigned)((M + GB_BM - 1) / GB_BM)), dim3(256), 0, (hipStream_t)stream, x, ldx, w.wp, w.oscale, bias,
                       gamma, beta, eps, y, ldy, M, K, w.guard());
    CHECK_LAUNCH();
    return 0;
}

template <bool F16>
static int gb_windows(const float *feat, int Bimg, int Hf, int Wf, int C, const int32_t *img_ids, const int32_t *cell_ids, int nwin, int wc, int stride, int win,
                      const float *zero_row, const void *packed_w, const float *bias, const float *window_bias, float *y, int ldy, int N, void *stream)
{
    if (!feat || !img_ids || !cell_ids || !zero_row || !packed_w || !y || Bimg <= 0 || Hf <= 0 || Wf <= 0 || C <= 0 || (C % 64) || nwin < 0 || wc <= 0 || stride <= 0 ||
        win <= 0 || N <= 0 || ldy < N || (((uintptr_t)feat | (uintptr_t)zero_row) & 15)) return MFR_E_ARG;
    if (nwin == 0) return 0;
    const long long Mll = (long long)nwin * win * win;
    if (Mll > 0x7fffffffll) return MFR_E_ARG;
    const int M = (int)Mll, K = C;
    const GbOperand<F16> w(packed_w, N, K);
    if (!w.dma_ok()) return MFR_E_ARG;
    const unsigned grid = gb_persistent_grid((M + GB_BM - 1) / GB_BM, (N + GB_BN - 1) / GB_BN);
    gb_launch_d<8, F16>((hipStream_t)stream, grid, feat, C, w, bias, y, ldy, M, N, K, 1, 0, 0, 0, nullptr, nullptr, 0.f,
                        GdWindows{img_ids, cell_ids, zero_row, window_bias, wc, stride, Hf, Wf, win});
    CHECK_LAUNCH();
    return 0;
}

extern "C" {

#ifdef GD_PROF
int mfr_gemm_split_profile(unsigned long long *out_host)
{
    return hipMemcpyFromSymbol(out_host, HIP_SYMBOL(gd_prof), sizeof(unsigned long long) * 256, 0, hipMemcpyDeviceToHost) == hipSuccess ? 0 : MFR_E_LAUNCH;
}
#endif

size_t mfr_gemm_bf16x3_pack_bytes(int N, int K)
{
    if (N <= 0 || K <= 0 || (K % GB_BK)) return 0;
    return gb_tile_bytes(N, K, false);
}

size_t mfr_gemm_f16x2_pack_bytes(int N, int K)
{
    if (N <= 0 || K <= 0 || (K % GB_BK)) return 0;
    return gb_tile_bytes(N, K, true) + (size_t)((N + GB_BN - 1) / GB_BN) * GB_BN * 4;
}

int mfr_gemm_bf16x3_pack(const float *w, int N, int K, void *packed, void *stream)
{
    if (!w || !packed || N <= 0 || K <= 0 || (K % GB_BK)) return MFR_E_ARG;
    const long long total = (long long)(gb_tile_bytes(N, K, false) / 16);
    hipLaunchKernelGGL((gb_pack_kernel<false>), dim3((unsigned)((total + 255) / 256)), dim3(256), 0, (hipStream_t)stream, w, N, K, total, (const float *)nullptr, (uint4 *)packed,
                       1.0f, K, 0ll, 0ll);
    CHECK_LAUNCH();
    return 0;
}

int mfr_gemm_f16x2_pack_batched(const float *w, int ldw, int nbatch, long long w_batch_stride, int N, int K, float out_mul, void *packed, void *stream)
{
    if (ldw < K || !w || !packed || N <= 0 || K <= 0 || (K % GB_BK) || nbatch <= 0 || nbatch > 65535 || !(out_mul > 0.f)) return MFR_E_ARG;
    const size_t tb = gb_tile_bytes(N, K, true);
    const long long total = (long long)(tb / 16);
    const int npad = (N + GB_BN - 1) / GB_BN * GB_BN;
    const size_t pbytes = tb + (size_t)npad * 4;
    float *oscale = (float *)((char *)packed + tb);
    hipLaunchKernelGGL(gb_scale_kernel, dim3((unsigned)npad, (unsigned)nbatch), dim3(64), 0, (hipStream_t)stream, w, N, K, npad, oscale, out_mul, ldw, w_batch_stride, (long long)(pbytes / 4));
    hipLaunchKernelGGL((gb_pack_kernel<true>), dim3((unsigned)((total + 255) / 256), (unsigned)nbatch), dim3(256), 0, (hipStream_t)stream, w, N, K, total, (const float *)oscale,
                       (uint4 *)packed, out_mul, ldw, w_batch_stride, (long long)(pbytes / 16));
    CHECK_LAUNCH();
    return 0;
}

int mfr_gemm_f16x2_pack(const float *w, int N, int K, void *packed, void *stream)
{
    return mfr_gemm_f16x2_pack_batched(w, K, 1, 0, N, K, 1.0f, packed, stream);
}

int mfr_gemm_bf16x3(const float *x, int ldx, const void *packed_w, const float *bias, float *y, int ldy, int M, int N, int K, int flags, void *stream)
{
    return gb_launch<false>(x, ldx, packed_w, bias, y, ldy, M, N, K, flags, stream);
}

int mfr_gemm_f16x2(const float *x, int ldx, const void *packed_w, const float *bias, float *y, int ldy, int M, int N, int K, int flags, void *stream)
{
    return gb_launch<true>(x, ldx, packed_w, bias, y, ldy, M, N, K, flags, stream);
}

int mfr_mlp_ln_f16x2(const float *x, int ldx, int K1, const void *packed_w1, const float *b1, const void *packed_w2, const float *b2, const float *gamma, const float *beta,
                     float eps, float *y, int ldy, int M, int accumulate, void *stream)
{
    return gb_mlp_ln<true>(x, ldx, K1, packed_w1, b1, packed_w2, b2, gamma, beta, eps, y, ldy, M, accumulate, stream);
}

int mfr_mlp_ln_bf16x3(const float *x, int ldx, int K1, const void *packed_w1, const float *b1, const void *packed_w2, const float *b2, const float *gamma, const float *beta,
                      float eps, float *y, int ldy, int M, int accumulate, void *stream)
{
    return gb_mlp_ln<false>(x, ldx, K1, packed_w1, b1, packed_w2, b2, gamma, beta, eps, y, ldy, M, accumulate, stream);
}

int mfr_gemm_f16x2_windows(const float *feat, int Bimg, int Hf, int Wf, int C, const int32_t *img_ids, const int32_t *cell_ids, int nwin, int wc, int stride, int win,
                           const float *zero_row, const void *packed_w, const float *bias, const float *window_bias, float *y, int ldy, int N, void *stream)
{
    return gb_windows<true>(feat, Bimg, Hf, Wf, C, img_ids, cell_ids, nwin, wc, stride, win, zero_row, packed_w, bias, window_bias, y, ldy, N, stream);
}

int mfr_gemm_bf16x3_windows(const float *feat, int Bimg, int Hf, int Wf, int C, const int32_t *img_ids, const int32_t *cell_ids, int nwin, int wc, int stride, int win,
                            const float *zero_row, const void *packed_w, const float *bias, const float *window_bias, float *y, int ldy, int N, void *stream)
{
    return gb_windows<false>(feat, Bimg, Hf, Wf, C, img_ids, cell_ids, nwin, wc, stride, win, zero_row, packed_w, bias, window_bias, y, ldy, N, stream);
}

int mfr_gemm_f16x2_ln(const float *x, int ldx, const void *packed_w, const float *bias, const float *gamma, const float *beta, float eps, float *y, int ldy,
                      int M, int N, int K, int accumulate, void *stream)
{
    if (!gamma || !beta) return MFR_E_ARG;
    return gb_launch<true>(x, ldx, packed_w, bias, y, ldy, M, N, K, accumulate ? 2 : 0, stream, 1, 0, 0, 0, gamma, beta, eps);
}

int mfr_gemm_bf16x3_ln(const float *x, int ldx, const void *packed_w, const float *bias, const float *gamma, const float *beta, float eps, float *y, int ldy,
                       int M, int N, int K, int accumulate, void *stream)
{
    if (!gamma || !beta) return MFR_E_ARG;
    return gb_launch<false>(x, ldx, packed_w, bias, y, ldy, M, N, K, accumulate ? 2 : 0, stream, 1, 0, 0, 0, gamma, beta, eps);
}

int mfr_gemm_f16x2_ln_gelu(const float *x, int ldx, const void *packed_w, const float *bias, const float *gamma, const float *beta, float eps, float *y, int ldy,
                           int M, int N, int K, void *stream)
{
    return gb_ln_gelu<true>(x, ldx, packed_w, bias, gamma, beta, eps, y, ldy, M, N, K, stream);
}

int mfr_gemm_bf16x3_ln_gelu(const float *x, int ldx, const void *packed_w, const float *bias, const float *gamma, const float *beta, float eps, float *y, int ldy,
                            int M, int N, int K, void *stream)
{
    return gb_ln_gelu<false>(x, ldx, packed_w, bias, gamma, beta, eps, y, ldy, M, N, K, stream);
}

int mfr_gemm_f16x2_batched(const float *x, int ldx, long long x_batch_stride, const void *packed_w, const float *bias, float *y, int ldy, long long y_batch_stride,
                           int nbatch, int M, int N, int K, int flags, void *stream)
{
    return gb_launch<true>(x, ldx, packed_w, bias, y, ldy, M, N, K, flags, stream, nbatch, x_batch_stride, (long long)mfr_gemm_f16x2_pack_bytes(N, K), y_batch_stride);
}

int mfr_conv_igemm_k(int Cin, int KH, int KW)
{
    if (Cin <= 0 || KH <= 0 || KW <= 0) return 0;
    return Cin == 1 ? (KH * KW + 31) / 32 * 32 : KH * KW * ((Cin + 31) / 32 * 32);
}

static int gb_conv_igemm(const float *x, const void *packed_w, const float *bias, float *y, int B, int Cin, int H, int W, int Cout, int KH, int KW,
                         int stride, int pad, int pad_hi, int relu, const float *lo, int Hl, int Wl, void *stream)
{
    if (!x || !packed_w || !y || B <= 0 || Cin <= 0 || H <= 0 || W <= 0 || Cout <= 0 || KH <= 0 || KW <= 0 || stride <= 0 || pad < 0 || pad_hi < 0) return MFR_E_ARG;
    if ((size_t)4 * ((Cin + 31) / 32 * 32) * H * W >= 0x7fffffffull) return MFR_E_ARG;
    const int Ho = (H + pad + pad_hi - KH) / stride + 1, Wo = (W + pad + pad_hi - KW) / stride + 1;
    if (Ho <= 0 || Wo <= 0) return MFR_E_ARG;
    if ((size_t)4 * Cout * Ho * Wo >= 0x40000000ull) return MFR_E_ARG;
    if (lo && (relu || Cin == 1 || Hl <= 0 || Wl <= 0 || Ho != 2 * Hl || Wo != 2 * Wl)) return MFR_E_ARG;
    const int K = mfr_conv_igemm_k(Cin, KH, KW), nkb = K / GB_BK, cblocks = (Cin + 31) / 32;
    const int nnb = (Cout + GB_BN - 1) / GB_BN, npt = (Ho * Wo + 127) / 128;
    const long long grid = (long long)B * npt * nnb;
    if (grid > 0x7fffffffll) return MFR_E_ARG;
    const size_t tb = gb_tile_bytes(Cout, K, true);
    const float *oscale = (const float *)((const char *)packed_w + tb);
    hipStream_t st = (hipStream_t)stream;
    const float rh = (lo && Ho > 1) ? (float)(Hl - 1) / (float)(Ho - 1) : 0.f, rw = (lo && Wo > 1) ? (float)(Wl - 1) / (float)(Wo - 1) : 0.f;
#define GB_GO(M_, R_, U_) hipLaunchKernelGGL((conv_igemm_f16x2_kernel<M_, R_, U_>), dim3((unsigned)grid), dim3(256), 0, st, x, (const uint4 *)packed_w, oscale, bias, y, B, Cin, H, W, Cout, Ho, Wo, KH, KW, stride, pad, nkb, cblocks, nnb, npt, mfr_guard_current(), lo, Hl, Wl, rh, rw)
    if (lo) GB_GO(0, false, true);
    else if (Cin == 1) { if (relu) GB_GO(1, true, false); else GB_GO(1, false, false); }
    else               { if (relu) GB_GO(0, true, false); else GB_GO(0, false, false); }
#undef GB_GO
    CHECK_LAUNCH();
    return 0;
}

int mfr_conv_igemm_f16x2(const float *x, const void *packed_w, const float *bias, float *y, int B, int Cin, int H, int W, int Cout, int KH, int KW,
                         int stride, int pad, int relu, void *stream)
{
    return gb_conv_igemm(x, packed_w, bias, y, B, Cin, H, W, Cout, KH, KW, stride, pad, pad, relu, nullptr, 0, 0, stream);
}

int mfr_conv_igemm_f16x2_pad(const float *x, const void *packed_w, const float *bias, float *y, int B, int Cin, int H, int W, int Cout, int KH, int KW,
                             int stride, int pad_lo, int pad_hi, int relu, void *stream)
{
    return gb_conv_igemm(x, packed_w, bias, y, B, Cin, H, W, Cout, KH, KW, stride, pad_lo, pad_hi, relu, nullptr, 0, 0, stream);
}

int mfr_conv_igemm_f16x2_upadd(const float *x, const void *packed_w, const float *bias, const float *lo, int Hl, int Wl, float *y, int B, int Cin, int H, int W,
                               int Cout, int KH, int KW, int stride, int pad, void *stream)
{
    if (!lo) return MFR_E_ARG;
    return gb_conv_igemm(x, packed_w, bias, y, B, Cin, H, W, Cout, KH, KW, stride, pad, pad, 0, lo, Hl, Wl, stream);
}

}
```

map-free-reloc_amd/csrc/split_f16.h:

```cpp
#pragma once
#include <hip/hip_runtime.h>

#define SF_LOW_SCALE 2048.0f

typedef _Float16 sf_f16x8 __attribute__((ext_vector_type(8)));

__device__ __forceinline__ void sf_split2(float x0, float x1, float S, unsigned &h, unsigned &l)
{
    float r0, r1;
    asm("v_cvt_pk_f16_f32 %0, %1, %2" : "=v"(h) : "v"(x0), "v"(x1));
    asm("v_fma_mix_f32 %0, %1, -1.0, %2 op_sel:[0,0,0] op_sel_hi:[1,0,0]" : "=v"(r0) : "v"(h), "v"(x0));
    asm("v_fma_mix_f32 %0, %1, -1.0, %2 op_sel:[1,0,0] op_sel_hi:[1,0,0]" : "=v"(r1) : "v"(h), "v"(x1));
    asm("v_fma_mixlo_f16 %0, %1, %2, 0 op_sel_hi:[0,0,0]" : "=v"(l) : "v"(r0), "s"(S));
    asm("v_fma_mixhi_f16 %0, %1, %2, 0 op_sel_hi:[0,0,0]" : "+v"(l) : "v"(r1), "s"(S));
}

__device__ __forceinline__ void sf_split_w(float ws, unsigned short &wh, unsigned short &wl, unsigned short &wq)
{
    const _Float16 h = (_Float16)ws;
    const _Float16 l = (_Float16)(ws - (float)h);
    const _Float16 q = (_Float16)((float)h * (1.0f / SF_LOW_SCALE));
    wh = __builtin_bit_cast(unsigned short, h);
    wl = __builtin_bit_cast(unsigned short, l);
    wq = __builtin_bit_cast(unsigned short, q);
}

__device__ __forceinline__ float sf_feature_scale(float maxabs)
{
    if (!(maxabs > 0.f) || !(maxabs < 3.0e38f)) return 1.0f;
    int e;
    (void)frexpf(maxabs, &e);
    int k = 15 - e;
    k = k > 126 ? 126 : (k < -126 ? -126 : k);
    return ldexpf(1.0f, k);
}

__device__ __forceinline__ void bf_split3(float x, unsigned &h, unsigned &m, unsigned &l)
{
    h = __float_as_uint(x);
    const float r = x - __uint_as_float(h & 0xffff0000u);
    m = __float_as_uint(r);
    l = __float_as_uint(r - __uint_as_float(m & 0xffff0000u));
}
__device__ __forceinline__ unsigned bf_pack_hi16(unsigned lo, unsigned hi) { return __builtin_amdgcn_perm(hi, lo, 0x07060302u); }

#define SF_MFMA(a, b, c) __builtin_amdgcn_mfma_f32_32x32x16_f16(__builtin_bit_cast(sf_f16x8, (a)), __builtin_bit_cast(sf_f16x8, (b)), (c), 0, 0, 0)
```

map-free-reloc_amd/nets/linear.py:

```python
import torch

from .. import _lib, options


class SplitLinear:
    def __init__(self, weight, bias=None, split=None):
        lib = _lib.load(require_gpu=True)
        self.split = split or options.get("SPLIT")
        if self.split not in ("f16x2", "bf16x3"):
            raise ValueError(f"SplitLinear: unknown split {self.split!r}")
        self._pack_bytes = getattr(lib, f"mfr_gemm_{self.split}_pack_bytes")
        self._pack = getattr(lib, f"mfr_gemm_{self.split}_pack")
        self._gemm = getattr(lib, f"mfr_gemm_{self.split}")
        self._gemm_ln = getattr(lib, f"mfr_gemm_{self.split}_ln")
        self.N, self.K = int(weight.shape[0]), int(weight.shape[1])
        nb = self._pack_bytes(self.N, self.K)
        if nb == 0:
            raise ValueError(f"SplitLinear: K = {self.K} must be a multiple of 32")
        w = weight.contiguous().float()
        self.packed = torch.empty(nb, dtype=torch.uint8, device=w.device)
        _lib.check(self._pack(_lib.ptr(w), self.N, self.K, _lib.ptr(self.packed), _lib.stream_ptr()), f"mfr_gemm_{self.split}_pack")
        self.bias = None if bias is None else bias.contiguous().float()

    def windows(self, feat_nhwc, img_ids, cell_ids, wc, stride, win, out, window_bias=None):
        Bimg, Hf, Wf, C = feat_nhwc.shape
        nwin = img_ids.numel()
        assert C == self.K and feat_nhwc.is_contiguous() and out.shape == (nwin * win * win, self.N) and out.stride(1) == 1
        assert img_ids.dtype == torch.int32 and cell_ids.dtype == torch.int32 and img_ids.is_contiguous() and cell_ids.is_contiguous()
        assert window_bias is None or (window_bias.shape == (nwin, self.N) and window_bias.is_contiguous())
        if getattr(self, "_zero_row", None) is None:
            self._zero_row = torch.zeros(self.K, dtype=torch.float32, device=feat_nhwc.device)
        lib = _lib.load()
        _lib.check(getattr(lib, f"mfr_gemm_{self.split}_windows")(_lib.ptr(feat_nhwc), Bimg, Hf, Wf, C, _lib.ptr(img_ids), _lib.ptr(cell_ids), nwin, wc, stride, win,
                                                                   _lib.ptr(self._zero_row), _lib.ptr(self.packed), _lib.ptr(self.bias), _lib.ptr(window_bias),
                                                                   out.data_ptr(), out.stride(0), self.N, _lib.stream_ptr()), f"mfr_gemm_{self.split}_windows")
        return out

    def ln_gelu(self, x, ln, out, eps=1e-5):
        assert self.N == 512 and x.dim() == 2 and x.shape[1] == self.K and x.stride(1) == 1 and x.dtype == torch.float32
        M = x.shape[0]
        assert out.shape == (M, 512) and out.stride(1) == 1
        fn = getattr(_lib.load(), f"mfr_gemm_{self.split}_ln_gelu")
        _lib.check(fn(x.data_ptr(), x.stride(0), _lib.ptr(self.packed), _lib.ptr(self.bias), _lib.ptr(ln[0]), _lib.ptr(ln[1]), float(eps), out.data_ptr(), out.stride(0),
                      M, self.N, self.K, _lib.stream_ptr()), f"mfr_gemm_{self.split}_ln_gelu")
        return out

    def ln_fusable(self):
        return self.N == 128 and self.K % 64 == 0

    def __call__(self, x, out=None, relu=False, accumulate=False, kernel_flag=0, ln=None, eps=1e-5):
        assert x.dim() == 2 and x.shape[1] == self.K and x.stride(1) == 1 and x.dtype == torch.float32
        M = x.shape[0]
        if out is None:
            assert not accumulate
            out = torch.empty(M, self.N, dtype=torch.float32, device=x.device)
        assert out.shape == (M, self.N) and out.stride(1) == 1
        if ln is not None:
            assert self.ln_fusable() and not relu and kernel_flag == 0
            _lib.check(self._gemm_ln(x.data_ptr(), x.stride(0), _lib.ptr(self.packed), _lib.ptr(self.bias), _lib.ptr(ln[0]), _lib.ptr(ln[1]), float(eps),
                                     out.data_ptr(), out.stride(0), M, self.N, self.K, 1 if accumulate else 0, _lib.stream_ptr()), f"mfr_gemm_{self.split}_ln")
            return out
        _lib.check(self._gemm(x.data_ptr(), x.stride(0), _lib.ptr(self.packed), _lib.ptr(self.bias), out.data_ptr(), out.stride(0),
                              M, self.N, self.K, (1 if relu else 0) | (2 if accumulate else 0) | kernel_flag, _lib.stream_ptr()), f"mfr_gemm_{self.split}")
        return out


class SplitBatchedNT:

    def __init__(self):
        self.lib = _lib.load(require_gpu=True)
        self.scratch = {}

    def __call__(self, x, w, out_mul=1.0, out=None):
        assert x.dim() == 3 and w.dim() == 3 and x.shape[0] == w.shape[0] and x.shape[2] == w.shape[2] and x.dtype == w.dtype == torch.float32
        nb, M, K = x.shape
        N = w.shape[1]
        assert x.stride(2) == 1 and w.stride(2) == 1
        per = self.lib.mfr_gemm_f16x2_pack_bytes(N, K)
        if per == 0:
            raise ValueError(f"SplitBatchedNT: K = {K} must be a multiple of 32")
        key = (nb, N, K, x.device)
        if key not in self.scratch:
            self.scratch[key] = torch.empty(nb * per, dtype=torch.uint8, device=x.device)
        pk = self.scratch[key]
        if out is None:
            out = torch.empty(nb, M, N, dtype=torch.float32, device=x.device)
        assert out.shape == (nb, M, N) and out.stride(2) == 1
        st = _lib.stream_ptr()
        _lib.check(self.lib.mfr_gemm_f16x2_pack_batched(w.data_ptr(), w.stride(1), nb, w.stride(0), N, K, float(out_mul), _lib.ptr(pk), st), "mfr_gemm_f16x2_pack_batched")
        _lib.check(self.lib.mfr_gemm_f16x2_batched(x.data_ptr(), x.stride(1), x.stride(0), _lib.ptr(pk), None, out.data_ptr(), out.stride(1), out.stride(0),
                                                   nb, M, N, K, 0, st), "mfr_gemm_f16x2_batched")
        return out


class FusedMlpLn:

    def __init__(self, lin1, lin2):
        assert lin1.split == lin2.split and lin1.N == 256 and lin2.N == 128 and lin2.K == 256 and lin1.K % 64 == 0
        self.l1, self.l2 = lin1, lin2
        self._fn = getattr(_lib.load(require_gpu=True), f"mfr_mlp_ln_{lin1.split}")

    def __call__(self, x, out, ln, accumulate=False, eps=1e-5):
        assert x.dim() == 2 and x.shape[1] == self.l1.K and x.stride(1) == 1 and x.dtype == torch.float32
        M = x.shape[0]
        assert out.shape == (M, 128) and out.stride(1) == 1
        _lib.check(self._fn(x.data_ptr(), x.stride(0), self.l1.K, _lib.ptr(self.l1.packed), _lib.ptr(self.l1.bias), _lib.ptr(self.l2.packed), _lib.ptr(self.l2.bias),
                            _lib.ptr(ln[0]), _lib.ptr(ln[1]), float(eps), out.data_ptr(), out.stride(0), M, 1 if accumulate else 0, _lib.stream_ptr()),
                   f"mfr_mlp_ln_{self.l1.split}")
        return out
```

map-free-reloc_amd/options.py:

```python
_SPEC = {
    "SPLIT": ("f16x2", ("f16x2", "bf16x3")),
    "CONV": ("wino", ("wino", "miopen")),
    "CONV_KERNEL": ("auto", ("auto", "split", "exact", "direct")),
    "CONV_TILE": ("auto", ("auto", "rows", "linear")),
    "FUSED_CONV1": (True, (False, True)),
    "FUSED_CONV_RELU": (False, (False, True)),
    "RPR_CONV": ("hip", ("hip", "miopen")),
    "RPR_CONV_BWD": ("lib", ("lib", "hip")),
    "RPR_CONV_ORDER": ("tap_inner", ("tap_inner", "tap_outer")),
    "RPR_WGRAD_SPLITS": (16, None),
    "RPR_ENCODER_NHWC": (False, (False, True)),
}
_VALUES = {k: v[0] for k, v in _SPEC.items()}
_EXPLICIT = set()


def names():
    return sorted(_SPEC)


def default(name):
    return _SPEC[name][0]


def get(name):
    return _VALUES[name]


def set(name, value):
    if name not in _SPEC:
        raise KeyError(f"unknown HIP option {name!r}; known: {names()}")
    dflt, allowed = _SPEC[name]
    if isinstance(dflt, bool):
        if isinstance(value, str):
            value = value.lower() in ("1", "true", "yes", "on")
        value = bool(value)
    elif isinstance(dflt, int):
        value = int(value)
        if value < 1:
            raise ValueError(f"HIP option {name}: must be >= 1")
    if allowed is not None and value not in allowed:
        raise ValueError(f"HIP option {name}={value!r}: allowed {allowed}")
    _VALUES[name] = value
    _EXPLICIT.add(name)


class override:

    def __init__(self, **kv):
        self.kv = kv

    def __enter__(self):
        self.saved = {k: (_VALUES[k], k in _EXPLICIT) for k in self.kv}
        for k, v in self.kv.items():
            set(k, v)
        return self

    def __exit__(self, *exc):
        for k, (v, ex) in self.saved.items():
            _VALUES[k] = v
            (_EXPLICIT.add if ex else _EXPLICIT.discard)(k)
        return False


def reset():
    for k, v in _SPEC.items():
        _VALUES[k] = v[0]
    _EXPLICIT.clear()


def apply_cfg(cfg):
    hip = cfg.HIP if "HIP" in cfg else {}
    for k in _SPEC:
        if k in hip:
            if k in _EXPLICIT and hip[k] == _SPEC[k][0]:
                continue
            explicit = k in _EXPLICIT
            set(k, hip[k])
            if not explicit:
                _EXPLICIT.discard(k)
```

Baseline: 1379.

## Add 16x16x32 f16 MFMA path for split GEMMs and make it default

Adds an alternative inner product in the split-f16 GEMM kernels that uses 16x16x32 f16 MFMA instructions with a 4x4 accumulator layout instead of 32x32x16. Fragment row mapping, epilogue stores, Y prefetch and guard checks are adapted to the new layout. The direct-DMA kernel raises its launch-bounds occupancy to 3 for plain epilogues. A GEMM_MFMA option, defaulting to 16x16x32, selects the path for linear, batched and window GEMMs. The smaller MFMA tile changes the issue pattern and register use, and it brings more instructions per tile and more scattered stores.

```diff
diff --git a/include/mfr_hip.h b/include/mfr_hip.h
--- a/include/mfr_hip.h
+++ b/include/mfr_hip.h
@@ -133,6 +133,8 @@
 int mfr_sp_sample_descriptors_ld(const float *dense_nhwc, int B, int Hc, int Wc, const float *kpts,
                                  const int32_t *n_kpts, int K, float *desc, int ldd, void *stream);
 
+#define MFR_GEMM_MFMA_16X16X32 16
+#define MFR_GEMM_WINDOWS_MFMA_16X16X32 0x10000
 size_t mfr_gemm_f16x2_pack_bytes(int N, int K);
 int mfr_gemm_f16x2_pack(const float *w, int N, int K, void *packed, void *stream);
 int mfr_gemm_f16x2(const float *x, int ldx, const void *packed_w, const float *bias, float *y, int ldy, int M, int N, int K, int flags, void *stream);
diff --git a/map-free-reloc_amd/csrc/gemm_split.hip b/map-free-reloc_amd/csrc/gemm_split.hip
--- a/map-free-reloc_amd/csrc/gemm_split.hip
+++ b/map-free-reloc_amd/csrc/gemm_split.hip
@@ -10,6 +10,7 @@
 
 typedef short bf16x8 __attribute__((ext_vector_type(8)));
 typedef float f32x16 __attribute__((ext_vector_type(16)));
+typedef float f32x4 __attribute__((ext_vector_type(4)));
 
 #define GB_BM 128
 #define GB_BN 128
@@ -62,7 +63,15 @@
     else     { GB_P4(1, 1); GB_P4(0, 2); GB_P4(2, 0); GB_P4(0, 1); GB_P4(1, 0); GB_P4(0, 0); }
 #undef GB_P4
 }
+__device__ __forceinline__ void gb_products(f32x4 (&acc)[4][4], const GbFrag (&a)[4][2], const GbFrag (&b)[3], int j)
+{
+#define GB_P16(ta, tb) do { _Pragma("unroll") for (int i = 0; i < 4; ++i) acc[i][j] = SF_MFMA16(a[i][ta].q, b[tb].q, acc[i][j]); } while (0)
+    GB_P16(1, 2); GB_P16(0, 1); GB_P16(0, 0);
+#undef GB_P16
+}
 #define GB_XT(F16) ((F16) ? 2 : 3)
+template <bool S16> struct GbAcc { typedef f32x16 T[2][2]; typedef unsigned OV[2][2][16]; };
+template <> struct GbAcc<true> { typedef f32x4 T[4][4]; typedef unsigned OV[4][4][4]; };
 
 #define GB_ACC_ROW(i, r) (32 * (i) + ((r) & 3) + 8 * ((r) >> 2))
 #define GB_TILE_ROW(base, i, r) ((base) + 32 * (i) + ((r) & 3) + 8 * ((r) >> 2) + 4 * (lane >> 5))
@@ -97,6 +106,32 @@
         _Pragma("unroll") for (int i = 0; i < 2; ++i) \
             _Pragma("unroll") for (int r = 0; r < 16; ++r) MFR_GUARD_ACC(chk, acc[i][0][r]); \
         mfr_guard_commit(guard, chk); } while (0)
+#define GB16_ACC_ROW(i, r) (16 * (i) + (r))
+#define GB16_TILE_ROW(base, i, r) ((base) + 16 * (i) + (r) + 4 * (lane >> 4))
+#define GB16_FRAG_ROW(w, kg_stride) ((lane >> 4) * (kg_stride) + 64 * (w) + (lane & 15))
+#define GBS_TILE_ROW(base, i, r) (S16 ? GB16_TILE_ROW(base, i, r) : GB_TILE_ROW(base, i, r))
+#define GBS_FRAG_ROW(w, kg_stride) (S16 ? GB16_FRAG_ROW(w, kg_stride) : GB_FRAG_ROW(w, kg_stride))
+#define GB16_WIDX_REG ((XT + t) * GB_TERM_UNITS + brow + 16 * i)
+#define GB16_MMA_KSTEP(acc, WIDX) do { \
+        GbFrag a[4][2]; \
+        _Pragma("unroll") for (int i = 0; i < 4; ++i) \
+            _Pragma("unroll") for (int t = 0; t < 2; ++t) a[i][t].q = lds[t * GB_TERM_UNITS + arow + 16 * i]; \
+        _Pragma("unroll") for (int i = 0; i < 4; ++i) {                        \
+            GbFrag b[3]; \
+            _Pragma("unroll") for (int t = 0; t < 2; ++t) b[t].q = lds[WIDX]; \
+            b[2].q = gb_wq(b[0].q); \
+            gb_products(acc, a, b, i); } } while (0)
+#define GBS_MMA_KSTEP(acc, WIDX, WIDX16) do { if constexpr (S16) GB16_MMA_KSTEP(acc, WIDX16); else GB_MMA_KSTEP(acc, false, WIDX); } while (0)
+#define GB16_ZERO(acc) do { \
+        _Pragma("unroll") for (int i = 0; i < 4; ++i) \
+            _Pragma("unroll") for (int jj = 0; jj < 4; ++jj) \
+                _Pragma("unroll") for (int r = 0; r < 4; ++r) acc[i][jj][r] = 0.f; } while (0)
+#define GBS_ZERO(acc) do { if constexpr (S16) GB16_ZERO(acc); else GB_ZERO(acc); } while (0)
+#define GB16_GUARD_ROWS(acc, chk) do { \
+        _Pragma("unroll") for (int i = 0; i < 4; ++i) \
+            _Pragma("unroll") for (int r = 0; r < 4; ++r) MFR_GUARD_ACC(chk, acc[i][0][r]); \
+        mfr_guard_commit(guard, chk); } while (0)
+#define GBS_GUARD_ROWS(acc, chk) do { if constexpr (S16) GB16_GUARD_ROWS(acc, chk); else GB_GUARD_ROWS(acc, chk); } while (0)
 #define GB_BATCH_OFFSETS() do { const size_t bz_ = blockIdx.y; X += bz_ * (size_t)xs; Wp += bz_ * (size_t)ws; Y += bz_ * (size_t)ys; if (F16) oscale += bz_ * (size_t)ws * 4; } while (0)
 
 __global__ void __launch_bounds__(64) gb_scale_kernel(const float *__restrict__ w, int N, int K, int npad, float *__restrict__ oscale, float out_mul,
@@ -143,11 +178,12 @@
     out[t] = make_uint4(bf_pack_hi16(word[0], word[1]), bf_pack_hi16(word[2], word[3]), bf_pack_hi16(word[4], word[5]), bf_pack_hi16(word[6], word[7]));
 }
 
-template <int FLAGS, bool F16>
+template <int FLAGS, bool F16, bool S16 = false>
 __global__ void __launch_bounds__(256, 2) gemm_split_kernel(const float *__restrict__ X, int ldx, const uint4 *__restrict__ Wp, const float *__restrict__ oscale,
                                                             const float *__restrict__ bias, float *__restrict__ Y, int ldy, int M, int N, int K, int nnb,
                                                             long long xs, long long ws, long long ys, int *guard)
 {
+    static_assert(F16 || !S16, "the 16x16x32 shape is f16x2 only");
     GB_BATCH_OFFSETS();
     constexpr int XT = GB_XT(F16);
     constexpr int WT = GB_WT(F16);
@@ -180,10 +216,10 @@
         const uint4 *wt_ = wtile + (size_t)(kb) * GB_W_TILE_UNITS(F16); \
         w0 = wt_[0]; w1 = wt_[256]; w2 = wt_[512]; w3 = wt_[768]; if (WT == 3) { w4 = wt_[1024]; w5 = wt_[1280]; } } while (0)
 
-    f32x16 acc[2][2];
-    GB_ZERO(acc);
-    const int arow = GB_FRAG_ROW(wm, GB_KG_STRIDE);
-    const int brow = GB_FRAG_ROW(wn, GB_KG_STRIDE);
+    typename GbAcc<S16>::T acc;
+    GBS_ZERO(acc);
+    const int arow = GBS_FRAG_ROW(wm, GB_KG_STRIDE);
+    const int brow = GBS_FRAG_ROW(wn, GB_KG_STRIDE);
 
     GB_GLOAD(0);
     for (int kb = 0; kb < nkb; ++kb) {
@@ -194,11 +230,34 @@
         __syncthreads();
         { const int kn = min(kb + 1, nkb - 1); GB_GLOAD(kn); }
         __builtin_amdgcn_sched_barrier(0);
-        GB_MMA_KSTEP(acc, false, GB_WIDX_REG);
+        GBS_MMA_KSTEP(acc, GB_WIDX_REG, GB16_WIDX_REG);
     }
 #undef GB_GLOAD
 
-    if (F16 && guard) { float chk = 0.f; GB_GUARD_ROWS(acc, chk); }
+    if (F16 && guard) { float chk = 0.f; GBS_GUARD_ROWS(acc, chk); }
+    if constexpr (S16) {
+#pragma unroll
+        for (int j = 0; j < 4; ++j) {
+            const int n = nb * GB_BN + 64 * wn + 16 * j + (lane & 15);
+            if (n >= N) continue;
+            const float bv = bias ? bias[n] : 0.f;
+            const float os = oscale[n];
+#pragma unroll
+            for (int i = 0; i < 4; ++i) {
+#pragma unroll
+                for (int r = 0; r < 4; ++r) {
+                    const int m = GB16_TILE_ROW(m0 + 64 * wm, i, r);
+                    if (m >= M) continue;
+                    float *yp = Y + (size_t)m * ldy + n;
+                    float v = __builtin_fmaf(acc[i][j][r], os, bv);
+                    if (FLAGS & 1) v = fmaxf(v, 0.f);
+                    if (FLAGS & 2) v += *yp;
+                    *yp = v;
+                }
+            }
+        }
+        return;
+    } else {
 #pragma unroll
     for (int j = 0; j < 2; ++j) {
         const int n = nb * GB_BN + 64 * wn + 32 * j + (lane & 31);
@@ -218,6 +277,7 @@
                 *yp = v;
             }
         }
+    }
     }
 }
 
@@ -234,12 +294,23 @@
     const __amdgpu_buffer_rsrc_t ry = __builtin_amdgcn_make_buffer_rsrc((void *)(Y + (size_t)m0 * ldy), 0, (int)((unsigned)min(GB_BM, M - m0) * rowb), MFR_RSRC_FLAGS); \
     const int n0 = (nb) * GB_BN + 64 * wn + (lane & 31); \
     const unsigned yoff = (unsigned)(64 * wm + 4 * (lane >> 5)) * rowb + 4u * (unsigned)n0
+#define GBS_YTILE(nb) \
+    const __amdgpu_buffer_rsrc_t ry = __builtin_amdgcn_make_buffer_rsrc((void *)(Y + (size_t)m0 * ldy), 0, (int)((unsigned)min(GB_BM, M - m0) * rowb), MFR_RSRC_FLAGS); \
+    const int n0 = (nb) * GB_BN + 64 * wn + (S16 ? (lane & 15) : (lane & 31)); \
+    const unsigned yoff = (unsigned)(64 * wm + 4 * (S16 ? (lane >> 4) : (lane >> 5))) * rowb + 4u * (unsigned)n0
+#define GB16_SOFF(i, r) ((unsigned)GB16_ACC_ROW(i, r) * rowb)
 #define GB_SOFF(i, r) ((unsigned)GB_ACC_ROW(i, r) * rowb)
 #define GB_PREFETCH_Y() do { \
         _Pragma("unroll") for (int jj = 0; jj < 2; ++jj) \
             _Pragma("unroll") for (int i = 0; i < 2; ++i) \
                 _Pragma("unroll") for (int r = 0; r < 16; ++r) \
                     ov[i][jj][r] = __builtin_amdgcn_raw_buffer_load_b32(ry, yoff + 128u * jj, GB_SOFF(i, r), 0); } while (0)
+#define GB16_PREFETCH_Y() do { \
+        _Pragma("unroll") for (int jj = 0; jj < 4; ++jj) \
+            _Pragma("unroll") for (int i = 0; i < 4; ++i) \
+                _Pragma("unroll") for (int r = 0; r < 4; ++r) \
+                    ov[i][jj][r] = __builtin_amdgcn_raw_buffer_load_b32(ry, yoff + 64u * jj, GB16_SOFF(i, r), 0); } while (0)
+#define GBS_PREFETCH_Y() do { if constexpr (S16) GB16_PREFETCH_Y(); else GB_PREFETCH_Y(); } while (0)
 #define GB_COLS() \
     const __amdgpu_buffer_rsrc_t rbias = __builtin_amdgcn_make_buffer_rsrc((void *)bias, 0, bias ? N * 4 : 0, MFR_RSRC_FLAGS); \
     const __amdgpu_buffer_rsrc_t rscale = __builtin_amdgcn_make_buffer_rsrc((void *)oscale, 0, F16 ? nnb * GB_BN * 4 : 0, MFR_RSRC_FLAGS)
@@ -248,6 +319,16 @@
     const float bv1 = __builtin_bit_cast(float, __builtin_amdgcn_raw_buffer_load_b32(rbias, 4u * (unsigned)n0 + 128u, 0, 0)); \
     const float os0 = __builtin_bit_cast(float, __builtin_amdgcn_raw_buffer_load_b32(rscale, 4u * (unsigned)n0, 0, 0)); \
     const float os1 = __builtin_bit_cast(float, __builtin_amdgcn_raw_buffer_load_b32(rscale, 4u * (unsigned)n0 + 128u, 0, 0))
+#define GBS_COLS_LOAD() \
+    const float bv0 = __builtin_bit_cast(float, __builtin_amdgcn_raw_buffer_load_b32(rbias, 4u * (unsigned)n0, 0, 0)); \
+    const float bv1 = __builtin_bit_cast(float, __builtin_amdgcn_raw_buffer_load_b32(rbias, 4u * (unsigned)n0 + (S16 ? 64u : 128u), 0, 0)); \
+    const float os0 = __builtin_bit_cast(float, __builtin_amdgcn_raw_buffer_load_b32(rscale, 4u * (unsigned)n0, 0, 0)); \
+    const float os1 = __builtin_bit_cast(float, __builtin_amdgcn_raw_buffer_load_b32(rscale, 4u * (unsigned)n0 + (S16 ? 64u : 128u), 0, 0)); \
+    const float bv2 = S16 ? __builtin_bit_cast(float, __builtin_amdgcn_raw_buffer_load_b32(rbias, 4u * (unsigned)n0 + 128u, 0, 0)) : 0.f; \
+    const float bv3 = S16 ? __builtin_bit_cast(float, __builtin_amdgcn_raw_buffer_load_b32(rbias, 4u * (unsigned)n0 + 192u, 0, 0)) : 0.f; \
+    const float os2 = S16 ? __builtin_bit_cast(float, __builtin_amdgcn_raw_buffer_load_b32(rscale, 4u * (unsigned)n0 + 128u, 0, 0)) : 0.f; \
+    const float os3 = S16 ? __builtin_bit_cast(float, __builtin_amdgcn_raw_buffer_load_b32(rscale, 4u * (unsigned)n0 + 192u, 0, 0)) : 0.f; \
+    (void)bv2; (void)bv3; (void)os2; (void)os3
 __device__ __forceinline__ void gb_xload(const float *&lx0, const float *&lx1, float4 &p0, float4 &p1, float4 &q0, float4 &q1)
 {
     p0 = *(const float4 *)lx0; p1 = *(const float4 *)(lx0 + 4); q0 = *(const float4 *)lx1; q1 = *(const float4 *)(lx1 + 4);
@@ -266,6 +347,19 @@
                     ROW_BIAS(v, i, jj, r); \
                     __builtin_amdgcn_raw_buffer_store_b32(__builtin_bit_cast(unsigned, v), ry, yoff + 128u * jj, GB_SOFF(i, r), 0); \
                 } } } while (0)
+#define GB16_STORE_PLAIN(acc, ROW_BIAS) do { \
+        _Pragma("unroll") for (int jj = 0; jj < 4; ++jj) { \
+            if (n0 + 16 * jj >= N) continue; \
+            const float bv = jj == 0 ? bv0 : jj == 1 ? bv1 : jj == 2 ? bv2 : bv3, os = jj == 0 ? os0 : jj == 1 ? os1 : jj == 2 ? os2 : os3; \
+            _Pragma("unroll") for (int i = 0; i < 4; ++i) \
+                _Pragma("unroll") for (int r = 0; r < 4; ++r) { \
+                    float v = __builtin_fmaf(acc[i][jj][r], os, bv); \
+                    if (FLAGS & 1) v = fmaxf(v, 0.f); \
+                    if (FLAGS & 2) v += __builtin_bit_cast(float, ov[i][jj][r]); \
+                    ROW_BIAS(v, i, jj, r); \
+                    __builtin_amdgcn_raw_buffer_store_b32(__builtin_bit_cast(unsigned, v), ry, yoff + 64u * jj, GB16_SOFF(i, r), 0); \
+                } } } while (0)
+#define GBS_STORE_PLAIN(acc, ROW_BIAS) do { if constexpr (S16) GB16_STORE_PLAIN(acc, ROW_BIAS); else GB_STORE_PLAIN(acc, ROW_BIAS); } while (0)
 #define GB_LN_ROW_SUMS(at) do { \
         _Pragma("unroll") for (int m = 1; m <= 16; m <<= 1) \
             _Pragma("unroll") for (int i = 0; i < 2; ++i) \
@@ -300,7 +394,7 @@
                 __builtin_amdgcn_raw_buffer_store_b32(__builtin_bit_cast(unsigned, y1), ry, yoff + 128u, GB_SOFF(i, r), 0); \
             } } while (0)
 
-template <int FLAGS, bool F16>
+template <int FLAGS, bool F16, bool S16 = false>
 __global__ void __launch_bounds__(256, 2) gemm_split_pk_kernel(const float *__restrict__ X, int ldx, const uint4 *__restrict__ Wp, const float *__restrict__ oscale,
                                                                const float *__restrict__ bias, float *__restrict__ Y, int ldy, int M, int N, int K, int nnb, int nmb,
                                                                long long xs, long long ws, long long ys, int *guard)
@@ -318,8 +412,9 @@
     int wdst[2 * WT];
 #pragma unroll
     for (int i = 0; i < 2 * WT; ++i) wdst[i] = gb_wdst(tid, i, XT);
-    const int arow = GB_FRAG_ROW(wm, GB_KG_STRIDE);
-    const int brow = GB_FRAG_ROW(wn, GB_KG_STRIDE);
+    static_assert(F16 || !S16, "the 16x16x32 shape is f16x2 only");
+    const int arow = GBS_FRAG_ROW(wm, GB_KG_STRIDE);
+    const int brow = GBS_FRAG_ROW(wn, GB_KG_STRIDE);
     const unsigned rowb = (unsigned)ldy * 4u;
     GB_COLS();
 
@@ -342,17 +437,17 @@
         if (++lk == nkb) { int jn = lj + per_xcd; if (jn < items) { GB_TILE(jn, mbn_, nbn_); (void)nbn_; if (mbn_ >= nmb) jn = items; } \
                            if (jn < items) lj = jn; load_tile_start(lj); } } while (0)
 
-    f32x16 acc[2][2];
-    unsigned ov[2][2][16];
+    typename GbAcc<S16>::T acc;
+    typename GbAcc<S16>::OV ov;
 
     load_tile_start(j);
     GB_PLOAD();
     for (;;) {
         GB_TILE(j, mb, nb);
         const int m0 = mb * GB_BM;
-        GB_YTILE(nb);
-        GB_COLS_LOAD();
-        GB_ZERO(acc);
+        GBS_YTILE(nb);
+        GBS_COLS_LOAD();
+        GBS_ZERO(acc);
 #define GB_PSTEP(LAST) do { \
             __syncthreads(); \
             gb_xsplit_store<F16>(lds, xa0, xa1, xdst[0]); gb_xsplit_store<F16>(lds, xb0, xb1, xdst[1]); \
@@ -360,14 +455,14 @@
             if (WT == 3) { lds[wdst[2 * WT - 2]] = w4; lds[wdst[2 * WT - 1]] = w5; } \
             __syncthreads(); \
             GB_PLOAD(); \
-            if ((LAST) && (FLAGS & 2)) GB_PREFETCH_Y(); \
+            if ((LAST) && (FLAGS & 2)) GBS_PREFETCH_Y(); \
             __builtin_amdgcn_sched_barrier(0); \
-            GB_MMA_KSTEP(acc, false, GB_WIDX_REG); } while (0)
+            GBS_MMA_KSTEP(acc, GB_WIDX_REG, GB16_WIDX_REG); } while (0)
         for (int kb = 0; kb < nkb - 1; ++kb) GB_PSTEP(false);
         GB_PSTEP(true);
 
-        if (F16 && guard) { float chk = 0.f; GB_GUARD_ROWS(acc, chk); }
-        GB_STORE_PLAIN(acc, GB_NO_ROW_BIAS);
+        if (F16 && guard) { float chk = 0.f; GBS_GUARD_ROWS(acc, chk); }
+        GBS_STORE_PLAIN(acc, GB_NO_ROW_BIAS);
         int jn = j + per_xcd;
         if (jn >= items) break;
         { GB_TILE(jn, mbn, nbn); (void)nbn; if (mbn >= nmb) break; }
@@ -403,6 +498,7 @@
             LOAD; \
         } } while (0)
 #define GD_WIDX(P) ((P) * WSTAGE + t * 512 + 2 * ks * 128 + brow + 32 * i)
+#define GD16_WIDX(P) ((P) * WSTAGE + t * 512 + brow + 16 * i)
 struct GdWindows {
     const int *img_ids, *cell_ids;
     const float *zero;
@@ -410,8 +506,8 @@
     int wc, stride, Hf, Wf, win;
 };
 
-template <int FLAGS, bool F16>
-__global__ void __launch_bounds__(256, 2) gemm_split_d_kernel(const float *__restrict__ X, int ldx, const uint4 *__restrict__ Wp, unsigned wp_bytes, const float *__restrict__ oscale,
+template <int FLAGS, bool F16, bool S16 = false>
+__global__ void __launch_bounds__(256, (S16 && !(FLAGS & 10)) ? 3 : 2) gemm_split_d_kernel(const float *__restrict__ X, int ldx, const uint4 *__restrict__ Wp, unsigned wp_bytes, const float *__restrict__ oscale,
                                                               const float *__restrict__ bias, float *__restrict__ Y, int ldy, int M, int N, int K, int nnb, int nmb,
                                                               long long xs, long long ws, long long ys, int *guard,
                                                               const float *__restrict__ ln_gamma, const float *__restrict__ ln_beta, float ln_eps, GdWindows wnd)
@@ -427,9 +523,10 @@
     GB_WALK();
     GB_WALK_NEXT();
 
+    static_assert((F16 && !(FLAGS & 4)) || !S16, "the 16x16x32 shape: f16x2, plain epilogue");
     GB_XSTAGE();
-    const int arow = GB_FRAG_ROW(wm, GB_KG_STRIDE);
-    const int brow = XT * GB_TERM_UNITS + GB_FRAG_ROW(wn, 128);
+    const int arow = GBS_FRAG_ROW(wm, GB_KG_STRIDE);
+    const int brow = XT * GB_TERM_UNITS + GBS_FRAG_ROW(wn, 128);
     const unsigned rowb = (unsigned)ldy * 4u;
     GB_COLS();
 
@@ -465,8 +562,8 @@
         gb_xload(lx0, lx1, p0, p1, q0, q1); \
         if (++lk == nkb) { lk = 0; lj = next_item(lj); x_tile_start(lj); } } while (0)
 
-    f32x16 acc[2][2];
-    unsigned ov[2][2][16];
+    typename GbAcc<S16>::T acc;
+    typename GbAcc<S16>::OV ov;
 #ifdef GD_PROF
     int pstep = 0;
 #define GD_PSTEP_INC ++pstep
@@ -480,13 +577,13 @@
         gb_xsplit_store<F16>(lds, p0, p1, xdst[0]); gb_xsplit_store<F16>(lds, q0, q1, xdst[1]); \
         wdma((P) ^ 1); GD_XLOAD(p0, p1, q0, q1); \
         GD_STAMP(2); \
-        if ((LAST) && (FLAGS & 2)) { GB_PREFETCH_Y(); GD_VMCNT(63); } \
+        if ((LAST) && (FLAGS & 2)) { GBS_PREFETCH_Y(); GD_VMCNT(63); } \
         else GD_VMCNT(8 + 2 * WT); \
         GD_STAMP(3); \
         __syncthreads(); \
         GD_STAMP(4); \
         __builtin_amdgcn_sched_barrier(0); \
-        GB_MMA_KSTEP(acc, false, GD_WIDX(P)); \
+        GBS_MMA_KSTEP(acc, GD_WIDX(P), GD16_WIDX(P)); \
         GD_PSTEP_INC; } while (0)
 
     x_tile_start(j);
@@ -496,13 +593,13 @@
     for (;;) {
         GB_TILE(j, mb, nb);
         const int m0 = mb * GB_BM;
-        GB_YTILE(nb);
-        GB_COLS_LOAD();
-        GB_ZERO(acc);
+        GBS_YTILE(nb);
+        GBS_COLS_LOAD();
+        GBS_ZERO(acc);
         for (int kb = 0; kb < nkb - 2; kb += 2) { GD_STEP(0, xa0, xa1, xb0, xb1, false); GD_STEP(1, xc0, xc1, xd0, xd1, false); }
         GD_STEP(0, xa0, xa1, xb0, xb1, false);
         GD_STEP(1, xc0, xc1, xd0, xd1, true);
-        if (F16 && guard) { float chk = 0.f; GB_GUARD_ROWS(acc, chk); }
+        if (F16 && guard) { float chk = 0.f; GBS_GUARD_ROWS(acc, chk); }
         if constexpr ((FLAGS & 4) != 0) {
             const float g0 = ln_gamma[n0], g1 = ln_gamma[n0 + 32], be0 = ln_beta[n0], be1 = ln_beta[n0 + 32];
             GB_STORE_LAYERNORM(acc, FLAGS & 2, bv0, bv1, os0, os1);
@@ -510,11 +607,11 @@
 #define GD_WINDOW_BIAS(v, i, jj, r) \
             if constexpr ((FLAGS & 8) != 0) { \
                 if (wnd.rgb) { \
-                    const int g = min(GB_TILE_ROW(m0 + 64 * wm, i, r), M - 1); \
-                    v += wnd.rgb[(size_t)(g / (wnd.win * wnd.win)) * N + n0 + 32 * jj]; \
+                    const int g = min(GBS_TILE_ROW(m0 + 64 * wm, i, r), M - 1); \
+                    v += wnd.rgb[(size_t)(g / (wnd.win * wnd.win)) * N + n0 + (S16 ? 16 : 32) * jj]; \
                 } \
             }
-            GB_STORE_PLAIN(acc, GD_WINDOW_BIAS);
+            GBS_STORE_PLAIN(acc, GD_WINDOW_BIAS);
 #undef GD_WINDOW_BIAS
         }
         const int jn = next_item(j);
@@ -988,12 +1085,12 @@
     const long long per_xcd = (long long)((nmb + 7) / 8) * nnb;
     return 8u * (unsigned)(per_xcd < cap ? per_xcd : cap);
 }
-template <int FLAGS, bool F16>
+template <int FLAGS, bool F16, bool S16 = false>
 static void gb_launch_d(hipStream_t st, unsigned grid, const float *x, int ldx, const GbOperand<F16> &w, const float *bias, float *y, int ldy, int M, int N, int K,
                         int nbatch = 1, long long xs = 0, long long ws = 0, long long ys = 0, const float *ln_gamma = nullptr, const float *ln_beta = nullptr,
                         float ln_eps = 0.f, const GdWindows &wnd = GdWindows{})
 {
-    hipLaunchKernelGGL((gemm_split_d_kernel<FLAGS, F16>), dim3(grid, (unsigned)nbatch), dim3(256), 0, st, x, ldx, w.wp, (unsigned)w.tb, w.oscale, bias, y, ldy, M, N, K,
+    hipLaunchKernelGGL((gemm_split_d_kernel<FLAGS, F16, S16>), dim3(grid, (unsigned)nbatch), dim3(256), 0, st, x, ldx, w.wp, (unsigned)w.tb, w.oscale, bias, y, ldy, M, N, K,
                        (N + GB_BN - 1) / GB_BN, (M + GB_BM - 1) / GB_BM, xs, ws, ys, GbOperand<F16>::guard(), ln_gamma, ln_beta, ln_eps, wnd);
 }
 
@@ -1015,9 +1112,10 @@
     }
     if (nbatch <= 0 || nbatch > 65535 || (ws_bytes & 15) || (xs & 3) || xs < 0 || ys < 0) return MFR_E_ARG;
     const long long ws = ws_bytes / 16;
-    if (!x || !packed_w || !y || M <= 0 || N <= 0 || K <= 0 || (K % GB_BK) || (ldx & 3) || ldx < K || ldy < N || flags < 0 || (flags & ~15) || (flags & 12) == 12) return MFR_E_ARG;
-    if (((uintptr_t)x & 15)) return MFR_E_ARG;
+    if (!x || !packed_w || !y || M <= 0 || N <= 0 || K <= 0 || (K % GB_BK) || (ldx & 3) || ldx < K || ldy < N || flags < 0 || (flags & ~31) || (flags & 12) == 12) return MFR_E_ARG;
+    if (((uintptr_t)x & 15) || (!F16 && (flags & MFR_GEMM_MFMA_16X16X32))) return MFR_E_ARG;
     const int f = flags & 3, one_tile = flags & 4;
+    const bool s16 = F16 && (flags & MFR_GEMM_MFMA_16X16X32);
     int pk = flags & 8;
     const GbOperand<F16> w(packed_w, N, K);
     if (!one_tile && !pk && ((K % 64) || !w.dma_ok())) pk = 8;
@@ -1025,20 +1123,22 @@
     const long long tiles = (long long)nmb * nnb;
     if (tiles > 0x7fffffffll) return MFR_E_ARG;
     const unsigned grid = gb_persistent_grid(nmb, nnb, (F16 && !(f & 2) && !pk) ? 96 : 64);
-#define GB_SW(GO) switch (f) { case 0: GO(0); break; case 1: GO(1); break; case 2: GO(2); break; default: GO(3); break; }
+#define GB_SW(GO) switch (f) { case 0: GB_SH(GO, 0); break; case 1: GB_SH(GO, 1); break; case 2: GB_SH(GO, 2); break; default: GB_SH(GO, 3); break; }
+#define GB_SH(GO, F) do { if (s16) GO(F, (F16 && true)); else GO(F, false); } while (0)
     if (one_tile) {
-#define GB_GO(F) hipLaunchKernelGGL((gemm_split_kernel<F, F16>), dim3((unsigned)tiles, (unsigned)nbatch), dim3(256), 0, st, x, ldx, w.wp, w.oscale, bias, y, ldy, M, N, K, nnb, xs, ws, ys, w.guard())
+#define GB_GO(F, S) hipLaunchKernelGGL((gemm_split_kernel<F, F16, S>), dim3((unsigned)tiles, (unsigned)nbatch), dim3(256), 0, st, x, ldx, w.wp, w.oscale, bias, y, ldy, M, N, K, nnb, xs, ws, ys, w.guard())
         GB_SW(GB_GO)
 #undef GB_GO
     } else if (pk) {
-#define GB_GO(F) hipLaunchKernelGGL((gemm_split_pk_kernel<F, F16>), dim3(grid, (unsigned)nbatch), dim3(256), 0, st, x, ldx, w.wp, w.oscale, bias, y, ldy, M, N, K, nnb, nmb, xs, ws, ys, w.guard())
+#define GB_GO(F, S) hipLaunchKernelGGL((gemm_split_pk_kernel<F, F16, S>), dim3(grid, (unsigned)nbatch), dim3(256), 0, st, x, ldx, w.wp, w.oscale, bias, y, ldy, M, N, K, nnb, nmb, xs, ws, ys, w.guard())
         GB_SW(GB_GO)
 #undef GB_GO
     } else {
-#define GB_GO(F) gb_launch_d<F, F16>(st, grid, x, ldx, w, bias, y, ldy, M, N, K, nbatch, xs, ws, ys)
+#define GB_GO(F, S) gb_launch_d<F, F16, S>(st, grid, x, ldx, w, bias, y, ldy, M, N, K, nbatch, xs, ws, ys)
         GB_SW(GB_GO)
 #undef GB_GO
     }
+#undef GB_SH
 #undef GB_SW
     CHECK_LAUNCH();
     return 0;
@@ -1080,6 +1180,9 @@
 {
     if (!feat || !img_ids || !cell_ids || !zero_row || !packed_w || !y || Bimg <= 0 || Hf <= 0 || Wf <= 0 || C <= 0 || (C % 64) || nwin < 0 || wc <= 0 || stride <= 0 ||
         win <= 0 || N <= 0 || ldy < N || (((uintptr_t)feat | (uintptr_t)zero_row) & 15)) return MFR_E_ARG;
+    const bool s16 = (win & MFR_GEMM_WINDOWS_MFMA_16X16X32) != 0;
+    win &= ~MFR_GEMM_WINDOWS_MFMA_16X16X32;
+    if (win <= 0 || (s16 && !F16)) return MFR_E_ARG;
     if (nwin == 0) return 0;
     const long long Mll = (long long)nwin * win * win;
     if (Mll > 0x7fffffffll) return MFR_E_ARG;
@@ -1087,8 +1190,9 @@
     const GbOperand<F16> w(packed_w, N, K);
     if (!w.dma_ok()) return MFR_E_ARG;
     const unsigned grid = gb_persistent_grid((M + GB_BM - 1) / GB_BM, (N + GB_BN - 1) / GB_BN);
-    gb_launch_d<8, F16>((hipStream_t)stream, grid, feat, C, w, bias, y, ldy, M, N, K, 1, 0, 0, 0, nullptr, nullptr, 0.f,
-                        GdWindows{img_ids, cell_ids, zero_row, window_bias, wc, stride, Hf, Wf, win});
+    const GdWindows wnd{img_ids, cell_ids, zero_row, window_bias, wc, stride, Hf, Wf, win};
+    if (s16) gb_launch_d<8, F16, (F16 && true)>((hipStream_t)stream, grid, feat, C, w, bias, y, ldy, M, N, K, 1, 0, 0, 0, nullptr, nullptr, 0.f, wnd);
+    else     gb_launch_d<8, F16>((hipStream_t)stream, grid, feat, C, w, bias, y, ldy, M, N, K, 1, 0, 0, 0, nullptr, nullptr, 0.f, wnd);
     CHECK_LAUNCH();
     return 0;
 }
diff --git a/map-free-reloc_amd/csrc/split_f16.h b/map-free-reloc_amd/csrc/split_f16.h
--- a/map-free-reloc_amd/csrc/split_f16.h
+++ b/map-free-reloc_amd/csrc/split_f16.h
@@ -45,3 +45,4 @@
 __device__ __forceinline__ unsigned bf_pack_hi16(unsigned lo, unsigned hi) { return __builtin_amdgcn_perm(hi, lo, 0x07060302u); }
 
 #define SF_MFMA(a, b, c) __builtin_amdgcn_mfma_f32_32x32x16_f16(__builtin_bit_cast(sf_f16x8, (a)), __builtin_bit_cast(sf_f16x8, (b)), (c), 0, 0, 0)
+#define SF_MFMA16(a, b, c) __builtin_amdgcn_mfma_f32_16x16x32_f16(__builtin_bit_cast(sf_f16x8, (a)), __builtin_bit_cast(sf_f16x8, (b)), (c), 0, 0, 0)
diff --git a/map-free-reloc_amd/nets/linear.py b/map-free-reloc_amd/nets/linear.py
--- a/map-free-reloc_amd/nets/linear.py
+++ b/map-free-reloc_amd/nets/linear.py
@@ -2,13 +2,24 @@
 
 from .. import _lib, options
 
+MFMA_16X16X32 = 16
+WINDOWS_MFMA_16X16X32 = 0x10000
+
+
+def _mfma16(mfma, split="f16x2"):
+    mfma = mfma or options.get("GEMM_MFMA")
+    if mfma not in ("32x32x16", "16x16x32"):
+        raise ValueError(f"unknown GEMM_MFMA {mfma!r}")
+    return split == "f16x2" and mfma == "16x16x32"
+
 
 class SplitLinear:
-    def __init__(self, weight, bias=None, split=None):
+    def __init__(self, weight, bias=None, split=None, mfma=None):
         lib = _lib.load(require_gpu=True)
         self.split = split or options.get("SPLIT")
         if self.split not in ("f16x2", "bf16x3"):
             raise ValueError(f"SplitLinear: unknown split {self.split!r}")
+        self.mfma16 = _mfma16(mfma, self.split)
         self._pack_bytes = getattr(lib, f"mfr_gemm_{self.split}_pack_bytes")
         self._pack = getattr(lib, f"mfr_gemm_{self.split}_pack")
         self._gemm = getattr(lib, f"mfr_gemm_{self.split}")
@@ -31,7 +42,8 @@
         if getattr(self, "_zero_row", None) is None:
             self._zero_row = torch.zeros(self.K, dtype=torch.float32, device=feat_nhwc.device)
         lib = _lib.load()
-        _lib.check(getattr(lib, f"mfr_gemm_{self.split}_windows")(_lib.ptr(feat_nhwc), Bimg, Hf, Wf, C, _lib.ptr(img_ids), _lib.ptr(cell_ids), nwin, wc, stride, win,
+        _lib.check(getattr(lib, f"mfr_gemm_{self.split}_windows")(_lib.ptr(feat_nhwc), Bimg, Hf, Wf, C, _lib.ptr(img_ids), _lib.ptr(cell_ids), nwin, wc, stride,
+                                                                   win + (WINDOWS_MFMA_16X16X32 if self.mfma16 else 0),
                                                                    _lib.ptr(self._zero_row), _lib.ptr(self.packed), _lib.ptr(self.bias), _lib.ptr(window_bias),
                                                                    out.data_ptr(), out.stride(0), self.N, _lib.stream_ptr()), f"mfr_gemm_{self.split}_windows")
         return out
@@ -61,15 +73,16 @@
                                      out.data_ptr(), out.stride(0), M, self.N, self.K, 1 if accumulate else 0, _lib.stream_ptr()), f"mfr_gemm_{self.split}_ln")
             return out
         _lib.check(self._gemm(x.data_ptr(), x.stride(0), _lib.ptr(self.packed), _lib.ptr(self.bias), out.data_ptr(), out.stride(0),
-                              M, self.N, self.K, (1 if relu else 0) | (2 if accumulate else 0) | kernel_flag, _lib.stream_ptr()), f"mfr_gemm_{self.split}")
+                              M, self.N, self.K, (1 if relu else 0) | (2 if accumulate else 0) | kernel_flag | (MFMA_16X16X32 if self.mfma16 else 0), _lib.stream_ptr()), f"mfr_gemm_{self.split}")
         return out
 
 
 class SplitBatchedNT:
 
-    def __init__(self):
+    def __init__(self, mfma=None):
         self.lib = _lib.load(require_gpu=True)
         self.scratch = {}
+        self.mfma16 = _mfma16(mfma)
 
     def __call__(self, x, w, out_mul=1.0, out=None):
         assert x.dim() == 3 and w.dim() == 3 and x.shape[0] == w.shape[0] and x.shape[2] == w.shape[2] and x.dtype == w.dtype == torch.float32
@@ -89,7 +102,7 @@
         st = _lib.stream_ptr()
         _lib.check(self.lib.mfr_gemm_f16x2_pack_batched(w.data_ptr(), w.stride(1), nb, w.stride(0), N, K, float(out_mul), _lib.ptr(pk), st), "mfr_gemm_f16x2_pack_batched")
         _lib.check(self.lib.mfr_gemm_f16x2_batched(x.data_ptr(), x.stride(1), x.stride(0), _lib.ptr(pk), None, out.data_ptr(), out.stride(1), out.stride(0),
-                                                   nb, M, N, K, 0, st), "mfr_gemm_f16x2_batched")
+                                                   nb, M, N, K, MFMA_16X16X32 if self.mfma16 else 0, st), "mfr_gemm_f16x2_batched")
         return out
 
 
diff --git a/map-free-reloc_amd/options.py b/map-free-reloc_amd/options.py
--- a/map-free-reloc_amd/options.py
+++ b/map-free-reloc_amd/options.py
@@ -3,6 +3,7 @@
     "CONV": ("wino", ("wino", "miopen")),
     "CONV_KERNEL": ("auto", ("auto", "split", "exact", "direct")),
     "CONV_TILE": ("auto", ("auto", "rows", "linear")),
+    "GEMM_MFMA": ("16x16x32", ("32x32x16", "16x16x32")),
     "FUSED_CONV1": (True, (False, True)),
     "FUSED_CONV_RELU": (False, (False, True)),
     "RPR_CONV": ("hip", ("hip", "miopen")),
```

After: 1391, median of 6. Within noise of the previous version (+0.9%).
